# unirestore/UniRestore

Measured on AMD Instinct MI355X. Metric: restored 512x512 images/sec @ 20 denoise steps (whole job), higher is better.
Workload: dtype bf16; 1 GPU; PIR 512x512 batch=8/GPU, 20 DDIM steps, bf16, hipGraph replay (BASELINE.json configs[1]; configs[2] shape for N=8); global_batch=8, per_gpu_batch=8, image=512, denoise_steps=20, parallelism=image-parallel dp1, weights=seeded random init (no checkpoints reachable)

## Files before the change

### unirestore_amd/csrc/tchain.hip

```cpp
#include "common.h"
#include "tchain_asm.inc"

namespace {

constexpr int TC_WB = 40960;
constexpr int TC_AUX = 4096;
constexpr int TC_TILE = TC_WB + TC_AUX;
constexpr int TC_SHARE = TC_TILE / 4;
constexpr int TC_NS = 3;
constexpr int TC_TOK = 128;
constexpr int TC_LDS = TC_NS * TC_TILE;

typedef __attribute__((address_space(3))) void* lptr_t;
typedef __attribute__((ext_vector_type(4))) unsigned u32x4;

#define TC_WAIT(N) asm volatile("s_waitcnt vmcnt(%0) lgkmcnt(0)" ::"n"(N) : "memory")

__device__ __forceinline__ float f4e(const float4& v, int e) { return e == 0 ? v.x : e == 1 ? v.y : e == 2 ? v.z : v.w; }

template <int NF> __device__ __forceinline__ void zero_acc(f32x16 (&acc)[NF]) {
#pragma unroll
  for (int f = 0; f < NF; ++f)
#pragma unroll
    for (int e = 0; e < 16; ++e) acc[f][e] = 0.f;
}

template <bool F16>
struct TChain {
  typedef typename Frag<F16>::type frag_t;
  unsigned lds0;
  u32x4 rs;
  int lane, wid, h, voff;
  int ti, ntiles, islot, cslot;
  int aoff[4];

#define TC_MFMA_BLOCK(ASM, ...)                                                              \
  do {                                                                                       \
    if constexpr (F16) asm volatile(ASM("v_mfma_f32_32x32x16_f16") __VA_ARGS__);              \
    else asm volatile(ASM("v_mfma_f32_32x32x16_bf16") __VA_ARGS__);                           \
  } while (0)

  __device__ __forceinline__ void init(unsigned char* sm, const unsigned char* stream, int nt) {
    lds0 = __builtin_amdgcn_readfirstlane((unsigned)(uintptr_t)(lptr_t)sm);
    lane = threadIdx.x & 63;
    wid = __builtin_amdgcn_readfirstlane(threadIdx.x >> 6);
    h = lane >> 5;
    voff = lane * 16;
    ti = islot = cslot = 0;
    ntiles = nt;
    const unsigned long long a = (unsigned long long)stream;
    rs[0] = __builtin_amdgcn_readfirstlane((unsigned)a);
    rs[1] = __builtin_amdgcn_readfirstlane((unsigned)(a >> 32) & 0xffffu);
    rs[2] = 0x7fffffffu;
    rs[3] = 0x00020000u;
#pragma unroll
    for (int s = 0; s < 4; ++s) aoff[s] = (lane & 31) * 128 + ((((2 * s + h) ^ ((lane >> 1) & 7))) << 4);
    dma_alone();
    dma_alone();
  }
  __device__ __forceinline__ void dma_args(unsigned& so, unsigned& ld) {
    const int t = ti < ntiles ? ti : ntiles - 1;
    so = (unsigned)t * TC_TILE + (unsigned)wid * TC_SHARE;
    ld = lds0 + (unsigned)islot * TC_TILE + (unsigned)wid * TC_SHARE;
    ++ti;
    islot = islot == TC_NS - 1 ? 0 : islot + 1;
  }
  __device__ __forceinline__ void dma_alone() {
    unsigned so, ld;
    dma_args(so, ld);
    asm volatile(TC_ASM_DMA : "+s"(so), "+s"(ld) : "v"(voff), "s"(rs) : "memory", "scc");
  }
  template <int EXTRA = 0>
  __device__ __forceinline__ unsigned acquire() {
    TC_WAIT(11 + EXTRA);
    __builtin_amdgcn_s_barrier();
    const unsigned slot = lds0 + (unsigned)cslot * TC_TILE;
    cslot = cslot == TC_NS - 1 ? 0 : cslot + 1;
    return slot;
  }
  __device__ __forceinline__ void drain() {
    TC_WAIT(0);
    __builtin_amdgcn_s_barrier();
  }

  template <bool Z>
  __device__ __forceinline__ void gemm_tile(f32x16 (&acc)[10], const frag_t& b0, const frag_t& b1, const frag_t& b2, const frag_t& b3, unsigned slot) {
    const unsigned a0 = slot + aoff[0], a1 = slot + aoff[1], a2 = slot + aoff[2], a3 = slot + aoff[3];
    frag_t t0, t1, t2, t3, t4, t5, t6;
    unsigned so, ld;
    dma_args(so, ld);
#define TC_GEMM_OPERANDS                                                                                                        \
    : "+a"(acc[0]), "+a"(acc[1]), "+a"(acc[2]), "+a"(acc[3]), "+a"(acc[4]), "+a"(acc[5]), "+a"(acc[6]), "+a"(acc[7]), "+a"(acc[8]),  \
      "+a"(acc[9]), "=&v"(t0), "=&v"(t1), "=&v"(t2), "=&v"(t3), "=&v"(t4), "=&v"(t5), "=&v"(t6), "+s"(so), "+s"(ld)       \
    : "v"(b0), "v"(b1), "v"(b2), "v"(b3), "v"(a0), "v"(a1), "v"(a2), "v"(a3), "v"(voff), "s"(rs), "s"(wid)                                  \
    : "memory", "scc"
    if constexpr (Z) TC_MFMA_BLOCK(TC_ASM_GEMM_N10_Z, TC_GEMM_OPERANDS);
    else TC_MFMA_BLOCK(TC_ASM_GEMM_N10, TC_GEMM_OPERANDS);
#undef TC_GEMM_OPERANDS
  }
  template <int EXTRA = 0>
  __device__ __forceinline__ unsigned gemm_stage(f32x16 (&acc)[10], const frag_t (&xb)[20]) {
    unsigned slot = acquire<EXTRA>();
    gemm_tile<true>(acc, xb[0], xb[1], xb[2], xb[3], slot);
#pragma unroll
    for (int kt = 1; kt < 5; ++kt) {
      slot = kt == 1 ? acquire<EXTRA>() : acquire();
      gemm_tile<false>(acc, xb[4 * kt], xb[4 * kt + 1], xb[4 * kt + 2], xb[4 * kt + 3], slot);
    }
    return slot;
  }
  __device__ __forceinline__ void ff1_tile(f32x16 (&ag)[2], const frag_t (&xb)[20], unsigned slot) {
    const unsigned a0 = slot + aoff[0], a1 = slot + aoff[1], a2 = slot + aoff[2], a3 = slot + aoff[3];
    frag_t t0, t1, t2, t3, t4, t5, t6;
    unsigned so, ld;
    dma_args(so, ld);
    TC_MFMA_BLOCK(TC_ASM_FF1_A,
                  : "+a"(ag[0]), "+a"(ag[1]), "=&v"(t0), "=&v"(t1), "=&v"(t2), "=&v"(t3), "=&v"(t4), "=&v"(t5), "=&v"(t6),
                    "+s"(so), "+s"(ld)
                  : "v"(xb[0]), "v"(xb[1]), "v"(xb[2]), "v"(xb[3]), "v"(xb[4]), "v"(xb[5]), "v"(xb[6]), "v"(xb[7]), "v"(xb[8]), "v"(xb[9]),
                    "v"(xb[10]), "v"(xb[11]), "v"(a0), "v"(a1), "v"(a2), "v"(a3), "v"(voff), "s"(rs), "s"(wid)
                  : "memory", "scc");
    TC_MFMA_BLOCK(TC_ASM_FF1_B,
                  : "+a"(ag[0]), "+a"(ag[1]), "=&v"(t0), "=&v"(t1), "=&v"(t2), "=&v"(t3), "=&v"(t4), "=&v"(t5), "=&v"(t6)
                  : "v"(xb[12]), "v"(xb[13]), "v"(xb[14]), "v"(xb[15]), "v"(xb[16]), "v"(xb[17]), "v"(xb[18]), "v"(xb[19]),
                    "v"(a0), "v"(a1), "v"(a2), "v"(a3)
                  : "memory");
  }

  __device__ __forceinline__ unsigned aux_base(unsigned slot) const { return slot + TC_WB + 32 * h; }
  template <int U>
  __device__ __forceinline__ void aux_ff1(unsigned slot, float4 (&q)[8]) const {
    asm volatile(TC_ASM_AUX_FF1
                 : "=&v"(q[0]), "=&v"(q[1]), "=&v"(q[2]), "=&v"(q[3]), "=&v"(q[4]), "=&v"(q[5]), "=&v"(q[6]), "=&v"(q[7])
                 : "v"(aux_base(slot)), "i"(64 * U)
                 : "memory");
  }
  template <int VEC, int F0>
  __device__ __forceinline__ void aux_vec4(unsigned slot, float4 (&q)[8]) const {
    asm volatile(TC_ASM_AUX_8
                 : "=&v"(q[0]), "=&v"(q[1]), "=&v"(q[2]), "=&v"(q[3]), "=&v"(q[4]), "=&v"(q[5]), "=&v"(q[6]), "=&v"(q[7])
                 : "v"(aux_base(slot)), "i"((VEC + 32 * F0) * 4)
                 : "memory");
  }

  __device__ __forceinline__ void att_s(f32x16& s0, f32x16& s1, f32x16& s2, const frag_t& q0, const frag_t& q1, const frag_t& q2, const frag_t& q3, unsigned slot) {
    const unsigned a0 = slot + aoff[0], a1 = slot + aoff[1], a2 = slot + aoff[2], a3 = slot + aoff[3];
    frag_t t0, t1, t2, t3, t4, t5, t6;
    unsigned so, ld;
    dma_args(so, ld);
    TC_MFMA_BLOCK(TC_ASM_ATT_S,
                  : "+a"(s0), "+a"(s1), "+a"(s2), "=&v"(t0), "=&v"(t1), "=&v"(t2), "=&v"(t3), "=&v"(t4), "=&v"(t5), "=&v"(t6), "+s"(so), "+s"(ld)
                  : "v"(q0), "v"(q1), "v"(q2), "v"(q3), "v"(a0), "v"(a1), "v"(a2), "v"(a3), "v"(voff), "s"(rs), "s"(wid)
                  : "memory", "scc");
  }
  __device__ __forceinline__ void att_pv(f32x16 (&o)[2], const frag_t (&pf)[5], unsigned slot) {
    const unsigned v0 = slot + 12288, v1 = slot + 20480;
    const unsigned a0 = v0 + aoff[0], a1 = v0 + aoff[1], a2 = v0 + aoff[2], a3 = v0 + aoff[3], a4 = v1 + aoff[0];
    frag_t t0, t1, t2, t3, t4, t5, t6;
    TC_MFMA_BLOCK(TC_ASM_ATT_PV,
                  : "+a"(o[0]), "+a"(o[1]), "=&v"(t0), "=&v"(t1), "=&v"(t2), "=&v"(t3), "=&v"(t4), "=&v"(t5), "=&v"(t6)
                  : "v"(pf[0]), "v"(pf[1]), "v"(pf[2]), "v"(pf[3]), "v"(pf[4]), "v"(a0), "v"(a1), "v"(a2), "v"(a3), "v"(a4)
                  : "memory");
  }
  template <int F>
  __device__ __forceinline__ void aux_bc(unsigned slot, float4 (&q)[8]) const {
    asm volatile(TC_ASM_AUX_BC8
                 : "=&v"(q[0]), "=&v"(q[1]), "=&v"(q[2]), "=&v"(q[3]), "=&v"(q[4]), "=&v"(q[5]), "=&v"(q[6]), "=&v"(q[7])
                 : "v"(aux_base(slot)), "i"(128 * F)
                 : "memory");
  }
  template <int FA>
  __device__ __forceinline__ void ln_pack(const f32x16& acc, unsigned slot, float mean, float rstd, frag_t& o0, frag_t& o1) const {
    float4 q[8];
    aux_bc<FA>(slot, q);
    const float mr = mean * rstd;
#pragma unroll
    for (int u = 0; u < 2; ++u) {
      float v[8];
#pragma unroll
      for (int e = 0; e < 8; ++e) v[e] = fmaf(rstd, acc[8 * u + e], fmaf(-mr, f4e(q[4 + 2 * u + (e >> 2)], e & 3), f4e(q[2 * u + (e >> 2)], e & 3)));
      if (u == 0) o0 = pack(v); else o1 = pack(v);
    }
  }

  static __device__ __forceinline__ void unpack(const frag_t& f, float (&o)[8]) { unpack8t<F16>(__builtin_bit_cast(uint4, f), o); }
  static __device__ __forceinline__ frag_t pack(const float (&v)[8]) { return __builtin_bit_cast(frag_t, pack8t<F16>(v)); }

  template <bool RES, bool GELU = false>
  __device__ __forceinline__ void bias_res_pack(const f32x16 (&acc)[10], unsigned slot, const frag_t (&res)[20], frag_t (&out)[20]) const {
    bias_res_pair<RES, GELU, 0>(acc, slot, res, out);
    bias_res_pair<RES, GELU, 1>(acc, slot, res, out);
    bias_res_pair<RES, GELU, 2>(acc, slot, res, out);
    bias_res_pair<RES, GELU, 3>(acc, slot, res, out);
    bias_res_pair<RES, GELU, 4>(acc, slot, res, out);
  }
  template <bool RES, bool GELU, int FP>
  __device__ __forceinline__ void bias_res_pair(const f32x16 (&acc)[10], unsigned slot, const frag_t (&res)[20], frag_t (&out)[20]) const {
    float4 q[8];
    aux_vec4<0, 2 * FP>(slot, q);
#pragma unroll
    for (int i = 0; i < 4; ++i) {
      const int f = 2 * FP + (i >> 1), u = i & 1;
      float r[8], v[8];
      if constexpr (RES) unpack(res[2 * f + u], r);
#pragma unroll
      for (int e = 0; e < 8; ++e) {
        v[e] = acc[f][8 * u + e] + f4e(q[2 * i + (e >> 2)], e & 3);
        if constexpr (GELU) v[e] = gelu_f(v[e]);
        if constexpr (RES) v[e] += r[e];
      }
      out[2 * f + u] = pack(v);
    }
  }
};

template <bool F16, int KS>
__device__ __forceinline__ void row_stats(const typename Frag<F16>::type (&x)[KS], float eps, float& mean, float& rstd) {
  float s = 0.f;
#pragma unroll
  for (int k = 0; k < KS; ++k) {
    float v[8];
    TChain<F16>::unpack(x[k], v);
    s += ((v[0] + v[1]) + (v[2] + v[3])) + ((v[4] + v[5]) + (v[6] + v[7]));
  }
  s += __shfl_xor(s, 32, 64);
  mean = s * (1.0f / (16 * KS));
  float q = 0.f;
#pragma unroll
  for (int k = 0; k < KS; ++k) {
    float v[8];
    TChain<F16>::unpack(x[k], v);
#pragma unroll
    for (int e = 0; e < 8; ++e) { const float d = v[e] - mean; q = fmaf(d, d, q); }
  }
  q += __shfl_xor(q, 32, 64);
  rstd = rsqrtf(q * (1.0f / (16 * KS)) + eps);
}

template <bool F16, int U>
__device__ __forceinline__ typename Frag<F16>::type ff1_epilogue(const TChain<F16>& tc, const f32x16 (&ag)[2], unsigned slot, float rstd, float mr) {
  float4 q[8];
  tc.template aux_ff1<U>(slot, q);
  float v[8];
#pragma unroll
  for (int e = 0; e < 8; ++e) {
    const float ba = f4e(q[e >> 2], e & 3), bg = f4e(q[2 + (e >> 2)], e & 3);
    const float ca = f4e(q[4 + (e >> 2)], e & 3), cg = f4e(q[6 + (e >> 2)], e & 3);
    const float a = fmaf(rstd, ag[0][8 * U + e], fmaf(-mr, ca, ba));
    const float g = fmaf(rstd, ag[1][8 * U + e], fmaf(-mr, cg, bg));
    v[e] = a * gelu_f(g);
  }
  return TChain<F16>::pack(v);
}

template <bool F16>
__device__ __forceinline__ unsigned ff_stage(TChain<F16>& tc, f32x16 (&acc)[10], f32x16 (&ag)[2], const typename Frag<F16>::type (&xb)[20],
                                             float mean, float rstd, int nchunk) {
  typedef typename Frag<F16>::type frag_t;
  const float mr = mean * rstd;
  unsigned last = 0;
  for (int c = 0; c < nchunk; ++c) {
    frag_t hid[4];
#pragma unroll
    for (int half = 0; half < 2; ++half) {
      const unsigned slot = tc.acquire();
      tc.ff1_tile(ag, xb, slot);
      hid[half * 2] = ff1_epilogue<F16, 0>(tc, ag, slot, rstd, mr);
      __builtin_amdgcn_sched_barrier(0);
      hid[half * 2 + 1] = ff1_epilogue<F16, 1>(tc, ag, slot, rstd, mr);
      __builtin_amdgcn_sched_barrier(0);
    }
    last = tc.acquire();
    tc.template gemm_tile<false>(acc, hid[0], hid[1], hid[2], hid[3], last);
  }
  return last;
}

template <bool F16>
__device__ __forceinline__ void load_frags(const uint16_t* __restrict__ base, long long tok, int ld, int h, typename Frag<F16>::type (&x)[20]) {
  const uint16_t* xp = base + tok * ld + 8 * h;
#pragma unroll
  for (int s = 0; s < 20; ++s) x[s] = *reinterpret_cast<const typename Frag<F16>::type*>(xp + 16 * s);
}
#define TC_STORE16(ptr, val) (*reinterpret_cast<uint4*>(ptr) = __builtin_bit_cast(uint4, val))
template <bool F16>
__device__ __forceinline__ void store_frags(uint16_t* __restrict__ base, long long tok, int ld, int h, const typename Frag<F16>::type (&x)[20]) {
  uint16_t* xp = base + tok * ld + 8 * h;
#pragma unroll
  for (int s = 0; s < 20; ++s) TC_STORE16(xp + 16 * s, x[s]);
}

struct MlpP {
  const unsigned char* stream;
  const uint16_t* x;
  uint16_t* y;
  int T, ldx, ldy, ntiles, hidden;
  float eps;
};

template <bool F16>
__global__ __launch_bounds__(256, 1) void tchain_mlp_kernel(const MlpP p) {
  typedef typename Frag<F16>::type frag_t;
  extern __shared__ __attribute__((aligned(16))) unsigned char smem[];
  TChain<F16> tc;
  tc.init(smem, p.stream, p.ntiles);
  const long long tok = (long long)blockIdx.x * TC_TOK + tc.wid * 32 + (tc.lane & 31);
  frag_t xb[20];
  load_frags<F16>(p.x, tok, p.ldx, tc.h, xb);
  float mean, rstd;
  row_stats<F16, 20>(xb, p.eps, mean, rstd);
  f32x16 acc[10], ag[2];
  zero_acc(acc);
  zero_acc(ag);
  const unsigned last = ff_stage<F16>(tc, acc, ag, xb, mean, rstd, p.hidden / 64);
#pragma unroll
  for (int s = 0; s < 20; ++s) asm volatile("" : "+v"(xb[s]));
  tc.template bias_res_pack<true>(acc, last, xb, xb);
  store_frags<F16>(p.y, tok, p.ldy, tc.h, xb);
  TC_WAIT(0);
}

template <bool F16>
int launch_mlp(const MlpP& p, hipStream_t s) {
  static ur::DeviceOnce attr_once;
  if (auto once_guard = attr_once.first()) {
    hipFuncSetAttribute(reinterpret_cast<const void*>(&tchain_mlp_kernel<F16>), hipFuncAttributeMaxDynamicSharedMemorySize, TC_LDS);
  }
  hipLaunchKernelGGL((tchain_mlp_kernel<F16>), dim3(p.T / TC_TOK), dim3(256), TC_LDS, s, p);
  return ur::check_launch("ur_ff_geglu_fused");
}


__device__ __forceinline__ long long token_again() {
  unsigned t = threadIdx.x;
  asm volatile("" : "+v"(t));
  return (long long)blockIdx.x * TC_TOK + (t >> 6) * 32 + (t & 31);
}

template <bool F16>
__device__ __forceinline__ void launder(typename Frag<F16>::type (&x)[20]) {
#pragma unroll
  for (int s = 0; s < 20; ++s) asm volatile("" : "+v"(x[s]));
}

template <bool F16, int F>
__device__ __forceinline__ void head_out(const TChain<F16>& tc, const f32x16 (&acc)[10], unsigned slot, float mean, float rstd, int part,
                                         uint16_t* op, typename Frag<F16>::type (&xb)[20]) {
  typedef typename Frag<F16>::type frag_t;
  frag_t o0, o1;
  tc.template ln_pack<F>(acc[F], slot, mean, rstd, o0, o1);
  if (part < 2) {
    TC_STORE16(op + 32 * F, o0);
    TC_STORE16(op + 32 * F + 16, o1);
  } else {
    xb[2 * F] = o0;
    xb[2 * F + 1] = o1;
  }
}

struct HeadP {
  const unsigned char* stream;
  const uint16_t* x;
  const float* ab;
  uint16_t* h0;
  uint16_t* q;
  uint16_t* k;
  uint16_t* vt;
  int T, tok_per_img, ntiles;
  float eps;
};

template <bool F16>
__global__ __launch_bounds__(256, 1) void tchain_head_kernel(const HeadP p) {
  typedef typename Frag<F16>::type frag_t;
  constexpr int C = 320;
  extern __shared__ __attribute__((aligned(16))) unsigned char smem[];
  TChain<F16> tc;
  tc.init(smem, p.stream, p.ntiles);
  const long long tok0 = (long long)blockIdx.x * TC_TOK;
  const long long tok = tok0 + tc.wid * 32 + (tc.lane & 31);
  const int img = (int)(tok0 / p.tok_per_img);
  frag_t xb[20];
  load_frags<F16>(p.x, tok, C, tc.h, xb);
  {
    const float* ap = p.ab + (long long)img * 2 * C + 8 * tc.h;
#pragma unroll
    for (int s = 0; s < 20; ++s) {
      const float4 a0 = *reinterpret_cast<const float4*>(ap + 16 * s), a1 = *reinterpret_cast<const float4*>(ap + 16 * s + 4);
      const float4 b0 = *reinterpret_cast<const float4*>(ap + C + 16 * s), b1 = *reinterpret_cast<const float4*>(ap + C + 16 * s + 4);
      float v[8];
      tc.unpack(xb[s], v);
      v[0] = fmaf(v[0], a0.x, b0.x); v[1] = fmaf(v[1], a0.y, b0.y); v[2] = fmaf(v[2], a0.z, b0.z); v[3] = fmaf(v[3], a0.w, b0.w);
      v[4] = fmaf(v[4], a1.x, b1.x); v[5] = fmaf(v[5], a1.y, b1.y); v[6] = fmaf(v[6], a1.z, b1.z); v[7] = fmaf(v[7], a1.w, b1.w);
      xb[s] = tc.pack(v);
      if ((s & 3) == 3) __builtin_amdgcn_sched_barrier(0);
    }
  }
  f32x16 acc[10];
  zero_acc(acc);
  unsigned slot = tc.gemm_stage(acc, xb);
  tc.template bias_res_pack<false>(acc, slot, xb, xb);
  store_frags<F16>(p.h0, token_again(), C, tc.h, xb);
  float mean, rstd;
  row_stats<F16, 20>(xb, p.eps, mean, rstd);
  launder<F16>(xb);
#pragma unroll
  for (int part = 0; part < 3; ++part) {
    slot = tc.template gemm_stage<20>(acc, xb);
    uint16_t* op = (part == 0 ? p.q : p.k) + token_again() * C + 8 * tc.h;
    head_out<F16, 0>(tc, acc, slot, mean, rstd, part, op, xb);
    head_out<F16, 1>(tc, acc, slot, mean, rstd, part, op, xb);
    head_out<F16, 2>(tc, acc, slot, mean, rstd, part, op, xb);
    head_out<F16, 3>(tc, acc, slot, mean, rstd, part, op, xb);
    head_out<F16, 4>(tc, acc, slot, mean, rstd, part, op, xb);
    head_out<F16, 5>(tc, acc, slot, mean, rstd, part, op, xb);
    head_out<F16, 6>(tc, acc, slot, mean, rstd, part, op, xb);
    head_out<F16, 7>(tc, acc, slot, mean, rstd, part, op, xb);
    head_out<F16, 8>(tc, acc, slot, mean, rstd, part, op, xb);
    head_out<F16, 9>(tc, acc, slot, mean, rstd, part, op, xb);
  }
  tc.drain();
  unsigned char* tr = smem + tc.wid * (C * 64);
  const int j = tc.lane & 31;
#pragma unroll
  for (int s = 0; s < 20; ++s) {
    const uint4 w = __builtin_bit_cast(uint4, xb[s]);
    const unsigned wv[4] = {w.x, w.y, w.z, w.w};
#pragma unroll
    for (int e = 0; e < 8; ++e) {
      const int c = 16 * s + 8 * tc.h + e;
      *reinterpret_cast<uint16_t*>(tr + c * 64 + j * 2) = (uint16_t)(wv[e >> 1] >> (16 * (e & 1)));
    }
  }
  __syncthreads();
  {
    const long long tin = tok0 - (long long)img * p.tok_per_img + tc.wid * 32;
    uint16_t* vp = p.vt + (long long)img * C * p.tok_per_img + tin + (tc.lane & 3) * 8;
#pragma unroll
    for (int i = 0; i < 20; ++i) {
      const int r = i * 16 + (tc.lane >> 2);
      *reinterpret_cast<uint4*>(vp + (long long)r * p.tok_per_img) = *reinterpret_cast<const uint4*>(tr + r * 64 + (tc.lane & 3) * 16);
    }
  }
}

template <bool F16>
__device__ __forceinline__ void gn_partials_of_tile(const TChain<F16>& tc, unsigned char* smem, const typename Frag<F16>::type (&y)[20],
                                                    float* gn_part, long long tok0, int tok_per_img) {
  typedef typename Frag<F16>::type frag_t;
  constexpr int C = 320, ROW = 2 * C + 16;
  unsigned char* yt = smem + (tc.wid * 32 + (tc.lane & 31)) * ROW + 16 * tc.h;
#pragma unroll
  for (int s = 0; s < 20; ++s) *reinterpret_cast<frag_t*>(yt + 32 * s) = y[s];
  __syncthreads();
  if (threadIdx.x < C / 2) {
    float s0 = 0.f, s1 = 0.f, q0 = 0.f, q1 = 0.f;
    for (int r = 0; r < TC_TOK; ++r) {
      const uint32_t w = *reinterpret_cast<const uint32_t*>(smem + r * ROW + threadIdx.x * 4);
      const float a = Act<F16>::lo(w), b = Act<F16>::hi(w);
      s0 += a; q0 = fmaf(a, a, q0); s1 += b; q1 = fmaf(b, b, q1);
    }
    const int img = (int)(tok0 / tok_per_img), parts = tok_per_img / TC_TOK;
    const int part = (int)((tok0 - (long long)img * tok_per_img) / TC_TOK);
    float* st = gn_part + (((long long)img * parts + part) * C + 2 * threadIdx.x) * 2;
    *reinterpret_cast<float4*>(st) = make_float4(s0, q0, s1, q1);
  }
}

struct CsceP {
  const unsigned char* stream;
  const uint16_t* x;
  const uint16_t* cond;
  uint16_t* y;
  float* gn_part;
  int T, tok_per_img, ntiles;
};

template <bool F16>
__global__ __launch_bounds__(256, 1) void tchain_csce_kernel(const CsceP p) {
  typedef typename Frag<F16>::type frag_t;
  constexpr int C = 320, CC = 256;
  extern __shared__ __attribute__((aligned(16))) unsigned char smem[];
  TChain<F16> tc;
  tc.init(smem, p.stream, p.ntiles);
  const long long tok0 = (long long)blockIdx.x * TC_TOK;
  const long long tok = tok0 + tc.wid * 32 + (tc.lane & 31);
  frag_t sb[20], hb[20];
  {
    const uint16_t* cp = p.cond + tok * CC + 8 * tc.h;
#pragma unroll
    for (int s = 0; s < 16; ++s) hb[s] = *reinterpret_cast<const frag_t*>(cp + 16 * s);
  }
  f32x16 acc[10];
  zero_acc(acc);
  unsigned slot = tc.acquire();
  tc.template gemm_tile<true>(acc, hb[0], hb[1], hb[2], hb[3], slot);
#pragma unroll
  for (int kt = 1; kt < 4; ++kt) {
    slot = tc.acquire();
    tc.template gemm_tile<false>(acc, hb[4 * kt], hb[4 * kt + 1], hb[4 * kt + 2], hb[4 * kt + 3], slot);
    if (kt == 2) load_frags<F16>(p.x, token_again(), C, tc.h, sb);
  }
  tc.template bias_res_pack<true>(acc, slot, sb, sb);
  slot = tc.gemm_stage(acc, sb);
  tc.template bias_res_pack<false, true>(acc, slot, hb, hb);
  slot = tc.gemm_stage(acc, hb);
  tc.template bias_res_pack<true>(acc, slot, sb, sb);
  store_frags<F16>(p.y, token_again(), C, tc.h, sb);
  tc.drain();
  if (p.gn_part) gn_partials_of_tile<F16>(tc, smem, sb, p.gn_part, tok0, p.tok_per_img);
}

struct TailP {
  const unsigned char* stream;
  const uint16_t* o1;
  const uint16_t* h0;
  const uint16_t* xres;
  uint16_t* y;
  float* gn_part;
  int T, tok_per_img, ntiles, hidden, tk;
  float eps, scale_log2e;
};

template <bool F16>
__global__ __launch_bounds__(256, 1) void tchain_tail_kernel(const TailP p) {
  typedef typename Frag<F16>::type frag_t;
  constexpr int C = 320;
  extern __shared__ __attribute__((aligned(16))) unsigned char smem[];
  TChain<F16> tc;
  tc.init(smem, p.stream, p.ntiles);
  const long long tok0 = (long long)blockIdx.x * TC_TOK;
  const long long tok = tok0 + tc.wid * 32 + (tc.lane & 31);
  frag_t hb[20], xq[20];
  load_frags<F16>(p.o1, tok, C, tc.h, xq);
  f32x16 acc[10], ag[2], sc2[1];
  zero_acc(acc);
  zero_acc(ag);
  zero_acc(sc2);
  unsigned slot = tc.acquire();
  tc.template gemm_tile<true>(acc, xq[0], xq[1], xq[2], xq[3], slot);
#pragma unroll
  for (int kt = 1; kt < 5; ++kt) {
    slot = tc.acquire();
    tc.template gemm_tile<false>(acc, xq[4 * kt], xq[4 * kt + 1], xq[4 * kt + 2], xq[4 * kt + 3], slot);
    if (kt == 3) load_frags<F16>(p.h0, token_again(), C, tc.h, hb);
  }
  tc.template bias_res_pack<true>(acc, slot, hb, hb);
  float mean, rstd;
  row_stats<F16, 20>(hb, p.eps, mean, rstd);
  launder<F16>(hb);
#pragma unroll
  for (int hd = 0; hd < 5; ++hd) {
    slot = tc.acquire();
    tc.ff1_tile(ag, hb, slot);
    frag_t qf[4];
    tc.template ln_pack<0>(ag[0], slot, mean, rstd, qf[0], qf[1]);
    tc.template ln_pack<1>(ag[1], slot, mean, rstd, qf[2], qf[3]);
    slot = tc.acquire();
    tc.att_s(ag[0], ag[1], sc2[0], qf[0], qf[1], qf[2], qf[3], slot);
    int lim = p.tk - 8 * tc.h;
    asm volatile("" : "+v"(lim));
    float mx = -INFINITY;
#pragma unroll
    for (int kf = 0; kf < 3; ++kf)
#pragma unroll
      for (int r = 0; r < 16; ++r) {
        const int key = 32 * kf + 16 * (r >> 3) + (r & 7);
        mx = fmaxf(mx, key < lim ? (kf < 2 ? ag[kf & 1][r] : sc2[0][r]) : -INFINITY);
      }
    mx = fmaxf(mx, __shfl_xor(mx, 32, 64));
    const float mc = mx * p.scale_log2e;
    float l = 0.f;
    frag_t pf[5];
#pragma unroll
    for (int ks = 0; ks < 5; ++ks) {
      float v[8];
#pragma unroll
      for (int e = 0; e < 8; ++e) {
        const int key = 16 * ks + e;
        const float sv = ks < 4 ? ag[(ks >> 1) & 1][8 * (ks & 1) + e] : sc2[0][e];
        v[e] = key < lim ? __builtin_amdgcn_exp2f(fmaf(sv, p.scale_log2e, -mc)) : 0.f;
        l += v[e];
      }
      pf[ks] = tc.pack(v);
    }
    l += __shfl_xor(l, 32, 64);
    tc.att_pv(ag, pf, slot);
    const float inv = __builtin_amdgcn_rcpf(l);
    frag_t of[4];
#pragma unroll
    for (int f = 0; f < 2; ++f)
#pragma unroll
      for (int u = 0; u < 2; ++u) {
        float v[8];
#pragma unroll
        for (int e = 0; e < 8; ++e) v[e] = ag[f][8 * u + e] * inv;
        of[2 * f + u] = tc.pack(v);
      }
    slot = tc.acquire();
    if (hd == 0) tc.template gemm_tile<true>(acc, of[0], of[1], of[2], of[3], slot);
    else tc.template gemm_tile<false>(acc, of[0], of[1], of[2], of[3], slot);
  }
  tc.template bias_res_pack<true>(acc, slot, hb, hb);
  row_stats<F16, 20>(hb, p.eps, mean, rstd);
  launder<F16>(hb);
  zero_acc(acc);
  slot = ff_stage<F16>(tc, acc, ag, hb, mean, rstd, p.hidden / 64);
  tc.template bias_res_pack<true>(acc, slot, hb, hb);
  slot = tc.gemm_stage(acc, hb);
  const long long tok2 = token_again();
  load_frags<F16>(p.xres, tok2, C, tc.h, xq);
  tc.template bias_res_pack<true>(acc, slot, xq, xq);
  store_frags<F16>(p.y, tok2, C, tc.h, xq);
  tc.drain();
  if (p.gn_part) gn_partials_of_tile<F16>(tc, smem, xq, p.gn_part, tok0, p.tok_per_img);
}

template <bool F16>
int launch_head(const HeadP& p, hipStream_t s) {
  static ur::DeviceOnce attr_once;
  if (auto once_guard = attr_once.first()) {
    hipFuncSetAttribute(reinterpret_cast<const void*>(&tchain_head_kernel<F16>), hipFuncAttributeMaxDynamicSharedMemorySize, TC_LDS);
  }
  hipLaunchKernelGGL((tchain_head_kernel<F16>), dim3(p.T / TC_TOK), dim3(256), TC_LDS, s, p);
  return ur::check_launch("ur_transformer_head_fused");
}
template <bool F16>
int launch_csce(const CsceP& p, hipStream_t s) {
  static ur::DeviceOnce attr_once;
  if (auto once_guard = attr_once.first()) {
    hipFuncSetAttribute(reinterpret_cast<const void*>(&tchain_csce_kernel<F16>), hipFuncAttributeMaxDynamicSharedMemorySize, TC_LDS);
  }
  hipLaunchKernelGGL((tchain_csce_kernel<F16>), dim3(p.T / TC_TOK), dim3(256), TC_LDS, s, p);
  return ur::check_launch("ur_csce_fused");
}
template <bool F16>
int launch_tail(const TailP& p, hipStream_t s) {
  static ur::DeviceOnce attr_once;
  if (auto once_guard = attr_once.first()) {
    hipFuncSetAttribute(reinterpret_cast<const void*>(&tchain_tail_kernel<F16>), hipFuncAttributeMaxDynamicSharedMemorySize, TC_LDS);
  }
  hipLaunchKernelGGL((tchain_tail_kernel<F16>), dim3(p.T / TC_TOK), dim3(256), TC_LDS, s, p);
  return ur::check_launch("ur_transformer_tail_fused");
}

}

extern "C" size_t ur_chain_tile_bytes(void) { return TC_TILE; }

extern "C" int ur_ff_geglu_fused(const void* x, const void* stream_w, size_t stream_bytes, void* y, long long T, int C, int hidden,
                                 int ldx, int ldy, float ln_eps, int dtype, ur_stream_t stream) {
  UR_REQUIRE(x && stream_w && y, "null pointer");
  UR_REQUIRE_DT(dtype);
  if (C != 320) return ur::fail(UR_E_UNSUPPORTED, "ur_ff_geglu_fused: C must be 320 (token-stationary chain: C/32 accumulator fragments per wave)");
  UR_REQUIRE(T > 0 && T % TC_TOK == 0 && T < (1ll << 31) / (long long)std::max(ldx, ldy), "T must be a positive multiple of 128");
  UR_REQUIRE(hidden > 0 && hidden % 64 == 0 && ldx % 8 == 0 && ldy % 8 == 0 && ldx >= C && ldy >= C, "hidden % 64, ld % 8");
  MlpP p = {};
  p.stream = (const unsigned char*)stream_w; p.x = (const uint16_t*)x; p.y = (uint16_t*)y;
  p.T = (int)T; p.ldx = ldx; p.ldy = ldy; p.hidden = hidden; p.ntiles = 3 * (hidden / 64); p.eps = ln_eps;
  UR_REQUIRE(stream_bytes >= (size_t)p.ntiles * TC_TILE, "weight stream too short");
  hipStream_t s = (hipStream_t)stream;
  const double flops = 2.0 * (double)T * C * hidden * 3.0;
  const double bytes = 2.0 * (double)T * C * 2 + (double)p.ntiles * TC_TILE;
  ur::ProfScope prof("chain_mlp", flops, bytes, s);
  UR_DT_SWITCH(dtype, return (launch_mlp<F16>(p, s)));
  return UR_OK;
}

extern "C" int ur_transformer_head_fused(const void* x, const float* gn_ab, const void* stream_w, size_t stream_bytes, void* h0, void* q,
                                         void* k, void* vt, long long T, int tokens_per_image, int C, float ln_eps, int dtype,
                                         ur_stream_t stream) {
  UR_REQUIRE(x && gn_ab && stream_w && h0 && q && k && vt, "null pointer");
  UR_REQUIRE_DT(dtype);
  if (C != 320) return ur::fail(UR_E_UNSUPPORTED, "ur_transformer_head_fused: C must be 320");
  UR_REQUIRE(T > 0 && tokens_per_image > 0 && tokens_per_image % TC_TOK == 0 && T % tokens_per_image == 0 && T * (long long)C < (1ll << 31),
             "tokens per image must be a multiple of 128 and divide T");
  HeadP p = {};
  p.stream = (const unsigned char*)stream_w; p.x = (const uint16_t*)x; p.ab = gn_ab; p.h0 = (uint16_t*)h0; p.q = (uint16_t*)q;
  p.k = (uint16_t*)k; p.vt = (uint16_t*)vt; p.T = (int)T; p.tok_per_img = tokens_per_image; p.ntiles = 20; p.eps = ln_eps;
  UR_REQUIRE(stream_bytes >= (size_t)p.ntiles * TC_TILE, "weight stream too short");
  hipStream_t s = (hipStream_t)stream;
  ur::ProfScope prof("chain_head", 2.0 * (double)T * C * C * 4.0, 2.0 * (double)T * C * 5 + (double)p.ntiles * TC_TILE, s);
  UR_DT_SWITCH(dtype, return (launch_head<F16>(p, s)));
  return UR_OK;
}

extern "C" int ur_transformer_tail_fused(const void* o1, const void* h0, const void* xres, const void* stream_w, size_t stream_bytes, void* y,
                                         float* gn_part, long long T, int tokens_per_image, int C, int hidden, int heads, int tk,
                                         float ln_eps, float attn_scale, int dtype, ur_stream_t stream) {
  UR_REQUIRE(o1 && h0 && xres && stream_w && y, "null pointer");
  UR_REQUIRE_DT(dtype);
  if (C != 320 || heads != 5 || tk < 1 || tk > 80)
    return ur::fail(UR_E_UNSUPPORTED, "ur_transformer_tail_fused: C must be 320 with 5 heads of 64 and at most 80 context tokens");
  UR_REQUIRE(T > 0 && tokens_per_image > 0 && tokens_per_image % TC_TOK == 0 && T % tokens_per_image == 0 && T * (long long)C < (1ll << 31),
             "tokens per image must be a multiple of 128 and divide T");
  UR_REQUIRE(hidden > 0 && hidden % 64 == 0, "hidden % 64");
  TailP p = {};
  p.stream = (const unsigned char*)stream_w; p.o1 = (const uint16_t*)o1; p.h0 = (const uint16_t*)h0; p.xres = (const uint16_t*)xres;
  p.y = (uint16_t*)y; p.gn_part = gn_part; p.T = (int)T; p.tok_per_img = tokens_per_image; p.hidden = hidden; p.tk = tk;
  p.ntiles = 25 + 3 * (hidden / 64); p.eps = ln_eps; p.scale_log2e = attn_scale * 1.4426950408889634f;
  UR_REQUIRE(stream_bytes >= (size_t)p.ntiles * TC_TILE, "weight stream too short");
  hipStream_t s = (hipStream_t)stream;
  const double flops = 2.0 * (double)T * C * (4.0 * C + 3.0 * hidden) + 4.0 * (double)T * tk * C;
  ur::ProfScope prof("chain_tail", flops, 2.0 * (double)T * C * 4 + (double)p.ntiles * TC_TILE, s);
  UR_DT_SWITCH(dtype, return (launch_tail<F16>(p, s)));
  return UR_OK;
}

extern "C" int ur_csce_fused(const void* x, const void* cond, const void* stream_w, size_t stream_bytes, void* y, float* gn_part, long long T,
                             int tokens_per_image, int C, int Ccond, int dtype, ur_stream_t stream) {
  UR_REQUIRE(x && cond && stream_w && y, "null pointer");
  UR_REQUIRE_DT(dtype);
  if (C != 320 || Ccond != 256) return ur::fail(UR_E_UNSUPPORTED, "ur_csce_fused: C must be 320 and the condition 256 channels wide");
  UR_REQUIRE(T > 0 && tokens_per_image > 0 && tokens_per_image % TC_TOK == 0 && T % tokens_per_image == 0 && T * (long long)C < (1ll << 31),
             "tokens per image must be a multiple of 128 and divide T");
  CsceP p = {};
  p.stream = (const unsigned char*)stream_w; p.x = (const uint16_t*)x; p.cond = (const uint16_t*)cond; p.y = (uint16_t*)y; p.gn_part = gn_part;
  p.T = (int)T; p.tok_per_img = tokens_per_image; p.ntiles = 14;
  UR_REQUIRE(stream_bytes >= (size_t)p.ntiles * TC_TILE, "weight stream too short");
  hipStream_t s = (hipStream_t)stream;
  ur::ProfScope prof("chain_csce", 2.0 * (double)T * C * (Ccond + 2.0 * C), 2.0 * (double)T * (2.0 * C + Ccond) + (double)p.ntiles * TC_TILE, s);
  UR_DT_SWITCH(dtype, return (launch_csce<F16>(p, s)));
  return UR_OK;
}
```

### unirestore_amd/csrc/tchain_asm.inc

```
#pragma once

#define TC_ASM_DMA \
  "s_mov_b32 m0, %1\n\t" \
  "s_nop 0\n\t" \
  "buffer_load_dwordx4 %2, %3, %0 offen offset:0 lds\n\t" \
  "buffer_load_dwordx4 %2, %3, %0 offen offset:1024 lds\n\t" \
  "buffer_load_dwordx4 %2, %3, %0 offen offset:2048 lds\n\t" \
  "buffer_load_dwordx4 %2, %3, %0 offen offset:3072 lds\n\t" \
  "s_add_u32 %0, %0, 0x1000\n\t" \
  "s_add_u32 %1, %1, 0x1000\n\t" \
  "s_mov_b32 m0, %1\n\t" \
  "s_nop 0\n\t" \
  "buffer_load_dwordx4 %2, %3, %0 offen offset:0 lds\n\t" \
  "buffer_load_dwordx4 %2, %3, %0 offen offset:1024 lds\n\t" \
  "buffer_load_dwordx4 %2, %3, %0 offen offset:2048 lds\n\t" \
  "buffer_load_dwordx4 %2, %3, %0 offen offset:3072 lds\n\t" \
  "s_add_u32 %0, %0, 0x1000\n\t" \
  "s_add_u32 %1, %1, 0x1000\n\t" \
  "s_mov_b32 m0, %1\n\t" \
  "s_nop 0\n\t" \
  "buffer_load_dwordx4 %2, %3, %0 offen offset:0 lds\n\t" \
  "buffer_load_dwordx4 %2, %3, %0 offen offset:1024 lds\n\t" \
  "buffer_load_dwordx4 %2, %3, %0 offen offset:2048 lds\n\t"

#define TC_ASM_GEMM_N10(MN) \
  "s_waitcnt lgkmcnt(0)\n\t" \
  "ds_read_b128 %10, %23 offset:0\n\t" \
  "ds_read_b128 %11, %23 offset:4096\n\t" \
  "ds_read_b128 %12, %23 offset:8192\n\t" \
  "ds_read_b128 %13, %23 offset:12288\n\t" \
  "ds_read_b128 %14, %23 offset:16384\n\t" \
  "ds_read_b128 %15, %23 offset:20480\n\t" \
  "ds_read_b128 %16, %23 offset:24576\n\t" \
  "s_waitcnt lgkmcnt(6)\n\t" \
  MN " %0, %10, %19, %0\n\t" \
  "ds_read_b128 %10, %23 offset:28672\n\t" \
  "s_waitcnt lgkmcnt(6)\n\t" \
  MN " %1, %11, %19, %1\n\t" \
  "ds_read_b128 %11, %23 offset:32768\n\t" \
  "s_waitcnt lgkmcnt(6)\n\t" \
  MN " %2, %12, %19, %2\n\t" \
  "ds_read_b128 %12, %23 offset:36864\n\t" \
  "s_waitcnt lgkmcnt(6)\n\t" \
  MN " %3, %13, %19, %3\n\t" \
  "ds_read_b128 %13, %24 offset:0\n\t" \
  "s_waitcnt lgkmcnt(6)\n\t" \
  MN " %4, %14, %19, %4\n\t" \
  "ds_read_b128 %14, %24 offset:4096\n\t" \
  "s_waitcnt lgkmcnt(6)\n\t" \
  MN " %5, %15, %19, %5\n\t" \
  "ds_read_b128 %15, %24 offset:8192\n\t" \
  "s_waitcnt lgkmcnt(6)\n\t" \
  MN " %6, %16, %19, %6\n\t" \
  "ds_read_b128 %16, %24 offset:12288\n\t" \
  "s_waitcnt lgkmcnt(6)\n\t" \
  MN " %7, %10, %19, %7\n\t" \
  "ds_read_b128 %10, %24 offset:16384\n\t" \
  "s_waitcnt lgkmcnt(6)\n\t" \
  MN " %8, %11, %19, %8\n\t" \
  "ds_read_b128 %11, %24 offset:20480\n\t" \
  "s_waitcnt lgkmcnt(6)\n\t" \
  MN " %9, %12, %19, %9\n\t" \
  "ds_read_b128 %12, %24 offset:24576\n\t" \
  "s_cmp_lg_u32 %29, 0\n\t" \
  "s_cbranch_scc1 .Ltc%=_0\n\t" \
  "s_mov_b32 m0, %18\n\t" \
  "s_nop 0\n\t" \
  "buffer_load_dwordx4 %27, %28, %17 offen offset:0 lds\n\t" \
  "buffer_load_dwordx4 %27, %28, %17 offen offset:1024 lds\n\t" \
  "buffer_load_dwordx4 %27, %28, %17 offen offset:2048 lds\n\t" \
  "buffer_load_dwordx4 %27, %28, %17 offen offset:3072 lds\n\t" \
  "s_add_u32 %17, %17, 0x1000\n\t" \
  "s_add_u32 %18, %18, 0x1000\n\t" \
  "s_mov_b32 m0, %18\n\t" \
  "s_nop 0\n\t" \
  "buffer_load_dwordx4 %27, %28, %17 offen offset:0 lds\n\t" \
  "buffer_load_dwordx4 %27, %28, %17 offen offset:1024 lds\n\t" \
  "buffer_load_dwordx4 %27, %28, %17 offen offset:2048 lds\n\t" \
  "buffer_load_dwordx4 %27, %28, %17 offen offset:3072 lds\n\t" \
  "s_add_u32 %17, %17, 0x1000\n\t" \
  "s_add_u32 %18, %18, 0x1000\n\t" \
  "s_mov_b32 m0, %18\n\t" \
  "s_nop 0\n\t" \
  "buffer_load_dwordx4 %27, %28, %17 offen offset:0 lds\n\t" \
  "buffer_load_dwordx4 %27, %28, %17 offen offset:1024 lds\n\t" \
  "buffer_load_dwordx4 %27, %28, %17 offen offset:2048 lds\n\t" \
  ".Ltc%=_0:\n\t" \
  "s_waitcnt lgkmcnt(6)\n\t" \
  MN " %0, %13, %20, %0\n\t" \
  "ds_read_b128 %13, %24 offset:28672\n\t" \
  "s_waitcnt lgkmcnt(6)\n\t" \
  MN " %1, %14, %20, %1\n\t" \
  "ds_read_b128 %14, %24 offset:32768\n\t" \
  "s_waitcnt lgkmcnt(6)\n\t" \
  MN " %2, %15, %20, %2\n\t" \
  "ds_read_b128 %15, %24 offset:36864\n\t" \
  "s_waitcnt lgkmcnt(6)\n\t" \
  MN " %3, %16, %20, %3\n\t" \
  "ds_read_b128 %16, %25 offset:0\n\t" \
  "s_waitcnt lgkmcnt(6)\n\t" \
  MN " %4, %10, %20, %4\n\t" \
  "ds_read_b128 %10, %25 offset:4096\n\t" \
  "s_waitcnt lgkmcnt(6)\n\t" \
  MN " %5, %11, %20, %5\n\t" \
  "ds_read_b128 %11, %25 offset:8192\n\t" \
  "s_waitcnt lgkmcnt(6)\n\t" \
  MN " %6, %12, %20, %6\n\t" \
  "ds_read_b128 %12, %25 offset:12288\n\t" \
  "s_waitcnt lgkmcnt(6)\n\t" \
  MN " %7, %13, %20, %7\n\t" \
  "ds_read_b128 %13, %25 offset:16384\n\t" \
  "s_waitcnt lgkmcnt(6)\n\t" \
  MN " %8, %14, %20, %8\n\t" \
  "ds_read_b128 %14, %25 offset:20480\n\t" \
  "s_waitcnt lgkmcnt(6)\n\t" \
  MN " %9, %15, %20, %9\n\t" \
  "ds_read_b128 %15, %25 offset:24576\n\t" \
  "s_cmp_lg_u32 %29, 1\n\t" \
  "s_cbranch_scc1 .Ltc%=_1\n\t" \
  "s_mov_b32 m0, %18\n\t" \
  "s_nop 0\n\t" \
  "buffer_load_dwordx4 %27, %28, %17 offen offset:0 lds\n\t" \
  "buffer_load_dwordx4 %27, %28, %17 offen offset:1024 lds\n\t" \
  "buffer_load_dwordx4 %27, %28, %17 offen offset:2048 lds\n\t" \
  "buffer_load_dwordx4 %27, %28, %17 offen offset:3072 lds\n\t" \
  "s_add_u32 %17, %17, 0x1000\n\t" \
  "s_add_u32 %18, %18, 0x1000\n\t" \
  "s_mov_b32 m0, %18\n\t" \
  "s_nop 0\n\t" \
  "buffer_load_dwordx4 %27, %28, %17 offen offset:0 lds\n\t" \
  "buffer_load_dwordx4 %27, %28, %17 offen offset:1024 lds\n\t" \
  "buffer_load_dwordx4 %27, %28, %17 offen offset:2048 lds\n\t" \
  "buffer_load_dwordx4 %27, %28, %17 offen offset:3072 lds\n\t" \
  "s_add_u32 %17, %17, 0x1000\n\t" \
  "s_add_u32 %18, %18, 0x1000\n\t" \
  "s_mov_b32 m0, %18\n\t" \
  "s_nop 0\n\t" \
  "buffer_load_dwordx4 %27, %28, %17 offen offset:0 lds\n\t" \
  "buffer_load_dwordx4 %27, %28, %17 offen offset:1024 lds\n\t" \
  "buffer_load_dwordx4 %27, %28, %17 offen offset:2048 lds\n\t" \
  ".Ltc%=_1:\n\t" \
  "s_waitcnt lgkmcnt(6)\n\t" \
  MN " %0, %16, %21, %0\n\t" \
  "ds_read_b128 %16, %25 offset:28672\n\t" \
  "s_waitcnt lgkmcnt(6)\n\t" \
  MN " %1, %10, %21, %1\n\t" \
  "ds_read_b128 %10, %25 offset:32768\n\t" \
  "s_waitcnt lgkmcnt(6)\n\t" \
  MN " %2, %11, %21, %2\n\t" \
  "ds_read_b128 %11, %25 offset:36864\n\t" \
  "s_waitcnt lgkmcnt(6)\n\t" \
  MN " %3, %12, %21, %3\n\t" \
  "ds_read_b128 %12, %26 offset:0\n\t" \
  "s_waitcnt lgkmcnt(6)\n\t" \
  MN " %4, %13, %21, %4\n\t" \
  "ds_read_b128 %13, %26 offset:4096\n\t" \
  "s_waitcnt lgkmcnt(6)\n\t" \
  MN " %5, %14, %21, %5\n\t" \
  "ds_read_b128 %14, %26 offset:8192\n\t" \
  "s_waitcnt lgkmcnt(6)\n\t" \
  MN " %6, %15, %21, %6\n\t" \
  "ds_read_b128 %15, %26 offset:12288\n\t" \
  "s_waitcnt lgkmcnt(6)\n\t" \
  MN " %7, %16, %21, %7\n\t" \
  "ds_read_b128 %16, %26 offset:16384\n\t" \
  "s_waitcnt lgkmcnt(6)\n\t" \
  MN " %8, %10, %21, %8\n\t" \
  "ds_read_b128 %10, %26 offset:20480\n\t" \
  "s_waitcnt lgkmcnt(6)\n\t" \
  MN " %9, %11, %21, %9\n\t" \
  "ds_read_b128 %11, %26 offset:24576\n\t" \
  "s_cmp_lg_u32 %29, 2\n\t" \
  "s_cbranch_scc1 .Ltc%=_2\n\t" \
  "s_mov_b32 m0, %18\n\t" \
  "s_nop 0\n\t" \
  "buffer_load_dwordx4 %27, %28, %17 offen offset:0 lds\n\t" \
  "buffer_load_dwordx4 %27, %28, %17 offen offset:1024 lds\n\t" \
  "buffer_load_dwordx4 %27, %28, %17 offen offset:2048 lds\n\t" \
  "buffer_load_dwordx4 %27, %28, %17 offen offset:3072 lds\n\t" \
  "s_add_u32 %17, %17, 0x1000\n\t" \
  "s_add_u32 %18, %18, 0x1000\n\t" \
  "s_mov_b32 m0, %18\n\t" \
  "s_nop 0\n\t" \
  "buffer_load_dwordx4 %27, %28, %17 offen offset:0 lds\n\t" \
  "buffer_load_dwordx4 %27, %28, %17 offen offset:1024 lds\n\t" \
  "buffer_load_dwordx4 %27, %28, %17 offen offset:2048 lds\n\t" \
  "buffer_load_dwordx4 %27, %28, %17 offen offset:3072 lds\n\t" \
  "s_add_u32 %17, %17, 0x1000\n\t" \
  "s_add_u32 %18, %18, 0x1000\n\t" \
  "s_mov_b32 m0, %18\n\t" \
  "s_nop 0\n\t" \
  "buffer_load_dwordx4 %27, %28, %17 offen offset:0 lds\n\t" \
  "buffer_load_dwordx4 %27, %28, %17 offen offset:1024 lds\n\t" \
  "buffer_load_dwordx4 %27, %28, %17 offen offset:2048 lds\n\t" \
  ".Ltc%=_2:\n\t" \
  "s_waitcnt lgkmcnt(6)\n\t" \
  MN " %0, %12, %22, %0\n\t" \
  "ds_read_b128 %12, %26 offset:28672\n\t" \
  "s_waitcnt lgkmcnt(6)\n\t" \
  MN " %1, %13, %22, %1\n\t" \
  "ds_read_b128 %13, %26 offset:32768\n\t" \
  "s_waitcnt lgkmcnt(6)\n\t" \
  MN " %2, %14, %22, %2\n\t" \
  "ds_read_b128 %14, %26 offset:36864\n\t" \
  "s_waitcnt lgkmcnt(6)\n\t" \
  MN " %3, %15, %22, %3\n\t" \
  "s_waitcnt lgkmcnt(5)\n\t" \
  MN " %4, %16, %22, %4\n\t" \
  "s_waitcnt lgkmcnt(4)\n\t" \
  MN " %5, %10, %22, %5\n\t" \
  "s_waitcnt lgkmcnt(3)\n\t" \
  MN " %6, %11, %22, %6\n\t" \
  "s_waitcnt lgkmcnt(2)\n\t" \
  MN " %7, %12, %22, %7\n\t" \
  "s_waitcnt lgkmcnt(1)\n\t" \
  MN " %8, %13, %22, %8\n\t" \
  "s_waitcnt lgkmcnt(0)\n\t" \
  MN " %9, %14, %22, %9\n\t" \
  "s_cmp_lg_u32 %29, 3\n\t" \
  "s_cbranch_scc1 .Ltc%=_3\n\t" \
  "s_mov_b32 m0, %18\n\t" \
  "s_nop 0\n\t" \
  "buffer_load_dwordx4 %27, %28, %17 offen offset:0 lds\n\t" \
  "buffer_load_dwordx4 %27, %28, %17 offen offset:1024 lds\n\t" \
  "buffer_load_dwordx4 %27, %28, %17 offen offset:2048 lds\n\t" \
  "buffer_load_dwordx4 %27, %28, %17 offen offset:3072 lds\n\t" \
  "s_add_u32 %17, %17, 0x1000\n\t" \
  "s_add_u32 %18, %18, 0x1000\n\t" \
  "s_mov_b32 m0, %18\n\t" \
  "s_nop 0\n\t" \
  "buffer_load_dwordx4 %27, %28, %17 offen offset:0 lds\n\t" \
  "buffer_load_dwordx4 %27, %28, %17 offen offset:1024 lds\n\t" \
  "buffer_load_dwordx4 %27, %28, %17 offen offset:2048 lds\n\t" \
  "buffer_load_dwordx4 %27, %28, %17 offen offset:3072 lds\n\t" \
  "s_add_u32 %17, %17, 0x1000\n\t" \
  "s_add_u32 %18, %18, 0x1000\n\t" \
  "s_mov_b32 m0, %18\n\t" \
  "s_nop 0\n\t" \
  "buffer_load_dwordx4 %27, %28, %17 offen offset:0 lds\n\t" \
  "buffer_load_dwordx4 %27, %28, %17 offen offset:1024 lds\n\t" \
  "buffer_load_dwordx4 %27, %28, %17 offen offset:2048 lds\n\t" \
  ".Ltc%=_3:\n\t" \
  "s_nop 15\n\t"

#define TC_ASM_GEMM_N10_Z(MN) \
  "s_waitcnt lgkmcnt(0)\n\t" \
  "ds_read_b128 %10, %23 offset:0\n\t" \
  "ds_read_b128 %11, %23 offset:4096\n\t" \
  "ds_read_b128 %12, %23 offset:8192\n\t" \
  "ds_read_b128 %13, %23 offset:12288\n\t" \
  "ds_read_b128 %14, %23 offset:16384\n\t" \
  "ds_read_b128 %15, %23 offset:20480\n\t" \
  "ds_read_b128 %16, %23 offset:24576\n\t" \
  "s_waitcnt lgkmcnt(6)\n\t" \
  MN " %0, %10, %19, 0\n\t" \
  "ds_read_b128 %10, %23 offset:28672\n\t" \
  "s_waitcnt lgkmcnt(6)\n\t" \
  MN " %1, %11, %19, 0\n\t" \
  "ds_read_b128 %11, %23 offset:32768\n\t" \
  "s_waitcnt lgkmcnt(6)\n\t" \
  MN " %2, %12, %19, 0\n\t" \
  "ds_read_b128 %12, %23 offset:36864\n\t" \
  "s_waitcnt lgkmcnt(6)\n\t" \
  MN " %3, %13, %19, 0\n\t" \
  "ds_read_b128 %13, %24 offset:0\n\t" \
  "s_waitcnt lgkmcnt(6)\n\t" \
  MN " %4, %14, %19, 0\n\t" \
  "ds_read_b128 %14, %24 offset:4096\n\t" \
  "s_waitcnt lgkmcnt(6)\n\t" \
  MN " %5, %15, %19, 0\n\t" \
  "ds_read_b128 %15, %24 offset:8192\n\t" \
  "s_waitcnt lgkmcnt(6)\n\t" \
  MN " %6, %16, %19, 0\n\t" \
  "ds_read_b128 %16, %24 offset:12288\n\t" \
  "s_waitcnt lgkmcnt(6)\n\t" \
  MN " %7, %10, %19, 0\n\t" \
  "ds_read_b128 %10, %24 offset:16384\n\t" \
  "s_waitcnt lgkmcnt(6)\n\t" \
  MN " %8, %11, %19, 0\n\t" \
  "ds_read_b128 %11, %24 offset:20480\n\t" \
  "s_waitcnt lgkmcnt(6)\n\t" \
  MN " %9, %12, %19, 0\n\t" \
  "ds_read_b128 %12, %24 offset:24576\n\t" \
  "s_cmp_lg_u32 %29, 0\n\t" \
  "s_cbranch_scc1 .Ltc%=_0\n\t" \
  "s_mov_b32 m0, %18\n\t" \
  "s_nop 0\n\t" \
  "buffer_load_dwordx4 %27, %28, %17 offen offset:0 lds\n\t" \
  "buffer_load_dwordx4 %27, %28, %17 offen offset:1024 lds\n\t" \
  "buffer_load_dwordx4 %27, %28, %17 offen offset:2048 lds\n\t" \
  "buffer_load_dwordx4 %27, %28, %17 offen offset:3072 lds\n\t" \
  "s_add_u32 %17, %17, 0x1000\n\t" \
  "s_add_u32 %18, %18, 0x1000\n\t" \
  "s_mov_b32 m0, %18\n\t" \
  "s_nop 0\n\t" \
  "buffer_load_dwordx4 %27, %28, %17 offen offset:0 lds\n\t" \
  "buffer_load_dwordx4 %27, %28, %17 offen offset:1024 lds\n\t" \
  "buffer_load_dwordx4 %27, %28, %17 offen offset:2048 lds\n\t" \
  "buffer_load_dwordx4 %27, %28, %17 offen offset:3072 lds\n\t" \
  "s_add_u32 %17, %17, 0x1000\n\t" \
  "s_add_u32 %18, %18, 0x1000\n\t" \
  "s_mov_b32 m0, %18\n\t" \
  "s_nop 0\n\t" \
  "buffer_load_dwordx4 %27, %28, %17 offen offset:0 lds\n\t" \
  "buffer_load_dwordx4 %27, %28, %17 offen offset:1024 lds\n\t" \
  "buffer_load_dwordx4 %27, %28, %17 offen offset:2048 lds\n\t" \
  ".Ltc%=_0:\n\t" \
  "s_waitcnt lgkmcnt(6)\n\t" \
  MN " %0, %13, %20, %0\n\t" \
  "ds_read_b128 %13, %24 offset:28672\n\t" \
  "s_waitcnt lgkmcnt(6)\n\t" \
  MN " %1, %14, %20, %1\n\t" \
  "ds_read_b128 %14, %24 offset:32768\n\t" \
  "s_waitcnt lgkmcnt(6)\n\t" \
  MN " %2, %15, %20, %2\n\t" \
  "ds_read_b128 %15, %24 offset:36864\n\t" \
  "s_waitcnt lgkmcnt(6)\n\t" \
  MN " %3, %16, %20, %3\n\t" \
  "ds_read_b128 %16, %25 offset:0\n\t" \
  "s_waitcnt lgkmcnt(6)\n\t" \
  MN " %4, %10, %20, %4\n\t" \
  "ds_read_b128 %10, %25 offset:4096\n\t" \
  "s_waitcnt lgkmcnt(6)\n\t" \
  MN " %5, %11, %20, %5\n\t" \
  "ds_read_b128 %11, %25 offset:8192\n\t" \
  "s_waitcnt lgkmcnt(6)\n\t" \
  MN " %6, %12, %20, %6\n\t" \
  "ds_read_b128 %12, %25 offset:12288\n\t" \
  "s_waitcnt lgkmcnt(6)\n\t" \
  MN " %7, %13, %20, %7\n\t" \
  "ds_read_b128 %13, %25 offset:16384\n\t" \
  "s_waitcnt lgkmcnt(6)\n\t" \
  MN " %8, %14, %20, %8\n\t" \
  "ds_read_b128 %14, %25 offset:20480\n\t" \
  "s_waitcnt lgkmcnt(6)\n\t" \
  MN " %9, %15, %20, %9\n\t" \
  "ds_read_b128 %15, %25 offset:24576\n\t" \
  "s_cmp_lg_u32 %29, 1\n\t" \
  "s_cbranch_scc1 .Ltc%=_1\n\t" \
  "s_mov_b32 m0, %18\n\t" \
  "s_nop 0\n\t" \
  "buffer_load_dwordx4 %27, %28, %17 offen offset:0 lds\n\t" \
  "buffer_load_dwordx4 %27, %28, %17 offen offset:1024 lds\n\t" \
  "buffer_load_dwordx4 %27, %28, %17 offen offset:2048 lds\n\t" \
  "buffer_load_dwordx4 %27, %28, %17 offen offset:3072 lds\n\t" \
  "s_add_u32 %17, %17, 0x1000\n\t" \
  "s_add_u32 %18, %18, 0x1000\n\t" \
  "s_mov_b32 m0, %18\n\t" \
  "s_nop 0\n\t" \
  "buffer_load_dwordx4 %27, %28, %17 offen offset:0 lds\n\t" \
  "buffer_load_dwordx4 %27, %28, %17 offen offset:1024 lds\n\t" \
  "buffer_load_dwordx4 %27, %28, %17 offen offset:2048 lds\n\t" \
  "buffer_load_dwordx4 %27, %28, %17 offen offset:3072 lds\n\t" \
  "s_add_u32 %17, %17, 0x1000\n\t" \
  "s_add_u32 %18, %18, 0x1000\n\t" \
  "s_mov_b32 m0, %18\n\t" \
  "s_nop 0\n\t" \
  "buffer_load_dwordx4 %27, %28, %17 offen offset:0 lds\n\t" \
  "buffer_load_dwordx4 %27, %28, %17 offen offset:1024 lds\n\t" \
  "buffer_load_dwordx4 %27, %28, %17 offen offset:2048 lds\n\t" \
  ".Ltc%=_1:\n\t" \
  "s_waitcnt lgkmcnt(6)\n\t" \
  MN " %0, %16, %21, %0\n\t" \
  "ds_read_b128 %16, %25 offset:28672\n\t" \
  "s_waitcnt lgkmcnt(6)\n\t" \
  MN " %1, %10, %21, %1\n\t" \
  "ds_read_b128 %10, %25 offset:32768\n\t" \
  "s_waitcnt lgkmcnt(6)\n\t" \
  MN " %2, %11, %21, %2\n\t" \
  "ds_read_b128 %11, %25 offset:36864\n\t" \
  "s_waitcnt lgkmcnt(6)\n\t" \
  MN " %3, %12, %21, %3\n\t" \
  "ds_read_b128 %12, %26 offset:0\n\t" \
  "s_waitcnt lgkmcnt(6)\n\t" \
  MN " %4, %13, %21, %4\n\t" \
  "ds_read_b128 %13, %26 offset:4096\n\t" \
  "s_waitcnt lgkmcnt(6)\n\t" \
  MN " %5, %14, %21, %5\n\t" \
  "ds_read_b128 %14, %26 offset:8192\n\t" \
  "s_waitcnt lgkmcnt(6)\n\t" \
  MN " %6, %15, %21, %6\n\t" \
  "ds_read_b128 %15, %26 offset:12288\n\t" \
  "s_waitcnt lgkmcnt(6)\n\t" \
  MN " %7, %16, %21, %7\n\t" \
  "ds_read_b128 %16, %26 offset:16384\n\t" \
  "s_waitcnt lgkmcnt(6)\n\t" \
  MN " %8, %10, %21, %8\n\t" \
  "ds_read_b128 %10, %26 offset:20480\n\t" \
  "s_waitcnt lgkmcnt(6)\n\t" \
  MN " %9, %11, %21, %9\n\t" \
  "ds_read_b128 %11, %26 offset:24576\n\t" \
  "s_cmp_lg_u32 %29, 2\n\t" \
  "s_cbranch_scc1 .Ltc%=_2\n\t" \
  "s_mov_b32 m0, %18\n\t" \
  "s_nop 0\n\t" \
  "buffer_load_dwordx4 %27, %28, %17 offen offset:0 lds\n\t" \
  "buffer_load_dwordx4 %27, %28, %17 offen offset:1024 lds\n\t" \
  "buffer_load_dwordx4 %27, %28, %17 offen offset:2048 lds\n\t" \
  "buffer_load_dwordx4 %27, %28, %17 offen offset:3072 lds\n\t" \
  "s_add_u32 %17, %17, 0x1000\n\t" \
  "s_add_u32 %18, %18, 0x1000\n\t" \
  "s_mov_b32 m0, %18\n\t" \
  "s_nop 0\n\t" \
  "buffer_load_dwordx4 %27, %28, %17 offen offset:0 lds\n\t" \
  "buffer_load_dwordx4 %27, %28, %17 offen offset:1024 lds\n\t" \
  "buffer_load_dwordx4 %27, %28, %17 offen offset:2048 lds\n\t" \
  "buffer_load_dwordx4 %27, %28, %17 offen offset:3072 lds\n\t" \
  "s_add_u32 %17, %17, 0x1000\n\t" \
  "s_add_u32 %18, %18, 0x1000\n\t" \
  "s_mov_b32 m0, %18\n\t" \
  "s_nop 0\n\t" \
  "buffer_load_dwordx4 %27, %28, %17 offen offset:0 lds\n\t" \
  "buffer_load_dwordx4 %27, %28, %17 offen offset:1024 lds\n\t" \
  "buffer_load_dwordx4 %27, %28, %17 offen offset:2048 lds\n\t" \
  ".Ltc%=_2:\n\t" \
  "s_waitcnt lgkmcnt(6)\n\t" \
  MN " %0, %12, %22, %0\n\t" \
  "ds_read_b128 %12, %26 offset:28672\n\t" \
  "s_waitcnt lgkmcnt(6)\n\t" \
  MN " %1, %13, %22, %1\n\t" \
  "ds_read_b128 %13, %26 offset:32768\n\t" \
  "s_waitcnt lgkmcnt(6)\n\t" \
  MN " %2, %14, %22, %2\n\t" \
  "ds_read_b128 %14, %26 offset:36864\n\t" \
  "s_waitcnt lgkmcnt(6)\n\t" \
  MN " %3, %15, %22, %3\n\t" \
  "s_waitcnt lgkmcnt(5)\n\t" \
  MN " %4, %16, %22, %4\n\t" \
  "s_waitcnt lgkmcnt(4)\n\t" \
  MN " %5, %10, %22, %5\n\t" \
  "s_waitcnt lgkmcnt(3)\n\t" \
  MN " %6, %11, %22, %6\n\t" \
  "s_waitcnt lgkmcnt(2)\n\t" \
  MN " %7, %12, %22, %7\n\t" \
  "s_waitcnt lgkmcnt(1)\n\t" \
  MN " %8, %13, %22, %8\n\t" \
  "s_waitcnt lgkmcnt(0)\n\t" \
  MN " %9, %14, %22, %9\n\t" \
  "s_cmp_lg_u32 %29, 3\n\t" \
  "s_cbranch_scc1 .Ltc%=_3\n\t" \
  "s_mov_b32 m0, %18\n\t" \
  "s_nop 0\n\t" \
  "buffer_load_dwordx4 %27, %28, %17 offen offset:0 lds\n\t" \
  "buffer_load_dwordx4 %27, %28, %17 offen offset:1024 lds\n\t" \
  "buffer_load_dwordx4 %27, %28, %17 offen offset:2048 lds\n\t" \
  "buffer_load_dwordx4 %27, %28, %17 offen offset:3072 lds\n\t" \
  "s_add_u32 %17, %17, 0x1000\n\t" \
  "s_add_u32 %18, %18, 0x1000\n\t" \
  "s_mov_b32 m0, %18\n\t" \
  "s_nop 0\n\t" \
  "buffer_load_dwordx4 %27, %28, %17 offen offset:0 lds\n\t" \
  "buffer_load_dwordx4 %27, %28, %17 offen offset:1024 lds\n\t" \
  "buffer_load_dwordx4 %27, %28, %17 offen offset:2048 lds\n\t" \
  "buffer_load_dwordx4 %27, %28, %17 offen offset:3072 lds\n\t" \
  "s_add_u32 %17, %17, 0x1000\n\t" \
  "s_add_u32 %18, %18, 0x1000\n\t" \
  "s_mov_b32 m0, %18\n\t" \
  "s_nop 0\n\t" \
  "buffer_load_dwordx4 %27, %28, %17 offen offset:0 lds\n\t" \
  "buffer_load_dwordx4 %27, %28, %17 offen offset:1024 lds\n\t" \
  "buffer_load_dwordx4 %27, %28, %17 offen offset:2048 lds\n\t" \
  ".Ltc%=_3:\n\t" \
  "s_nop 15\n\t"

#define TC_ASM_FF1_A(MN) \
  "s_waitcnt lgkmcnt(0)\n\t" \
  "ds_read_b128 %2, %23 offset:0\n\t" \
  "ds_read_b128 %3, %23 offset:4096\n\t" \
  "ds_read_b128 %4, %24 offset:0\n\t" \
  "ds_read_b128 %5, %24 offset:4096\n\t" \
  "ds_read_b128 %6, %25 offset:0\n\t" \
  "ds_read_b128 %7, %25 offset:4096\n\t" \
  "ds_read_b128 %8, %26 offset:0\n\t" \
  "s_waitcnt lgkmcnt(6)\n\t" \
  MN " %0, %2, %11, 0\n\t" \
  "ds_read_b128 %2, %26 offset:4096\n\t" \
  "s_waitcnt lgkmcnt(6)\n\t" \
  MN " %1, %3, %11, 0\n\t" \
  "ds_read_b128 %3, %23 offset:8192\n\t" \
  "s_waitcnt lgkmcnt(6)\n\t" \
  MN " %0, %4, %12, %0\n\t" \
  "ds_read_b128 %4, %23 offset:12288\n\t" \
  "s_waitcnt lgkmcnt(6)\n\t" \
  MN " %1, %5, %12, %1\n\t" \
  "ds_read_b128 %5, %24 offset:8192\n\t" \
  "s_waitcnt lgkmcnt(6)\n\t" \
  MN " %0, %6, %13, %0\n\t" \
  "ds_read_b128 %6, %24 offset:12288\n\t" \
  "s_waitcnt lgkmcnt(6)\n\t" \
  MN " %1, %7, %13, %1\n\t" \
  "ds_read_b128 %7, %25 offset:8192\n\t" \
  "s_cmp_lg_u32 %29, 0\n\t" \
  "s_cbranch_scc1 .Ltc%=_0\n\t" \
  "s_mov_b32 m0, %10\n\t" \
  "s_nop 0\n\t" \
  "buffer_load_dwordx4 %27, %28, %9 offen offset:0 lds\n\t" \
  "buffer_load_dwordx4 %27, %28, %9 offen offset:1024 lds\n\t" \
  "buffer_load_dwordx4 %27, %28, %9 offen offset:2048 lds\n\t" \
  "buffer_load_dwordx4 %27, %28, %9 offen offset:3072 lds\n\t" \
  "s_add_u32 %9, %9, 0x1000\n\t" \
  "s_add_u32 %10, %10, 0x1000\n\t" \
  "s_mov_b32 m0, %10\n\t" \
  "s_nop 0\n\t" \
  "buffer_load_dwordx4 %27, %28, %9 offen offset:0 lds\n\t" \
  "buffer_load_dwordx4 %27, %28, %9 offen offset:1024 lds\n\t" \
  "buffer_load_dwordx4 %27, %28, %9 offen offset:2048 lds\n\t" \
  "buffer_load_dwordx4 %27, %28, %9 offen offset:3072 lds\n\t" \
  "s_add_u32 %9, %9, 0x1000\n\t" \
  "s_add_u32 %10, %10, 0x1000\n\t" \
  "s_mov_b32 m0, %10\n\t" \
  "s_nop 0\n\t" \
  "buffer_load_dwordx4 %27, %28, %9 offen offset:0 lds\n\t" \
  "buffer_load_dwordx4 %27, %28, %9 offen offset:1024 lds\n\t" \
  "buffer_load_dwordx4 %27, %28, %9 offen offset:2048 lds\n\t" \
  ".Ltc%=_0:\n\t" \
  "s_waitcnt lgkmcnt(6)\n\t" \
  MN " %0, %8, %14, %0\n\t" \
  "ds_read_b128 %8, %25 offset:12288\n\t" \
  "s_waitcnt lgkmcnt(6)\n\t" \
  MN " %1, %2, %14, %1\n\t" \
  "ds_read_b128 %2, %26 offset:8192\n\t" \
  "s_waitcnt lgkmcnt(6)\n\t" \
  MN " %0, %3, %15, %0\n\t" \
  "ds_read_b128 %3, %26 offset:12288\n\t" \
  "s_waitcnt lgkmcnt(6)\n\t" \
  MN " %1, %4, %15, %1\n\t" \
  "ds_read_b128 %4, %23 offset:16384\n\t" \
  "s_waitcnt lgkmcnt(6)\n\t" \
  MN " %0, %5, %16, %0\n\t" \
  "ds_read_b128 %5, %23 offset:20480\n\t" \
  "s_waitcnt lgkmcnt(6)\n\t" \
  MN " %1, %6, %16, %1\n\t" \
  "ds_read_b128 %6, %24 offset:16384\n\t" \
  "s_cmp_lg_u32 %29, 1\n\t" \
  "s_cbranch_scc1 .Ltc%=_1\n\t" \
  "s_mov_b32 m0, %10\n\t" \
  "s_nop 0\n\t" \
  "buffer_load_dwordx4 %27, %28, %9 offen offset:0 lds\n\t" \
  "buffer_load_dwordx4 %27, %28, %9 offen offset:1024 lds\n\t" \
  "buffer_load_dwordx4 %27, %28, %9 offen offset:2048 lds\n\t" \
  "buffer_load_dwordx4 %27, %28, %9 offen offset:3072 lds\n\t" \
  "s_add_u32 %9, %9, 0x1000\n\t" \
  "s_add_u32 %10, %10, 0x1000\n\t" \
  "s_mov_b32 m0, %10\n\t" \
  "s_nop 0\n\t" \
  "buffer_load_dwordx4 %27, %28, %9 offen offset:0 lds\n\t" \
  "buffer_load_dwordx4 %27, %28, %9 offen offset:1024 lds\n\t" \
  "buffer_load_dwordx4 %27, %28, %9 offen offset:2048 lds\n\t" \
  "buffer_load_dwordx4 %27, %28, %9 offen offset:3072 lds\n\t" \
  "s_add_u32 %9, %9, 0x1000\n\t" \
  "s_add_u32 %10, %10, 0x1000\n\t" \
  "s_mov_b32 m0, %10\n\t" \
  "s_nop 0\n\t" \
  "buffer_load_dwordx4 %27, %28, %9 offen offset:0 lds\n\t" \
  "buffer_load_dwordx4 %27, %28, %9 offen offset:1024 lds\n\t" \
  "buffer_load_dwordx4 %27, %28, %9 offen offset:2048 lds\n\t" \
  ".Ltc%=_1:\n\t" \
  "s_waitcnt lgkmcnt(6)\n\t" \
  MN " %0, %7, %17, %0\n\t" \
  "ds_read_b128 %7, %24 offset:20480\n\t" \
  "s_waitcnt lgkmcnt(6)\n\t" \
  MN " %1, %8, %17, %1\n\t" \
  "ds_read_b128 %8, %25 offset:16384\n\t" \
  "s_waitcnt lgkmcnt(6)\n\t" \
  MN " %0, %2, %18, %0\n\t" \
  "ds_read_b128 %2, %25 offset:20480\n\t" \
  "s_waitcnt lgkmcnt(6)\n\t" \
  MN " %1, %3, %18, %1\n\t" \
  "ds_read_b128 %3, %26 offset:16384\n\t" \
  "s_waitcnt lgkmcnt(6)\n\t" \
  MN " %0, %4, %19, %0\n\t" \
  "ds_read_b128 %4, %26 offset:20480\n\t" \
  "s_waitcnt lgkmcnt(6)\n\t" \
  MN " %1, %5, %19, %1\n\t" \
  "s_cmp_lg_u32 %29, 2\n\t" \
  "s_cbranch_scc1 .Ltc%=_2\n\t" \
  "s_mov_b32 m0, %10\n\t" \
  "s_nop 0\n\t" \
  "buffer_load_dwordx4 %27, %28, %9 offen offset:0 lds\n\t" \
  "buffer_load_dwordx4 %27, %28, %9 offen offset:1024 lds\n\t" \
  "buffer_load_dwordx4 %27, %28, %9 offen offset:2048 lds\n\t" \
  "buffer_load_dwordx4 %27, %28, %9 offen offset:3072 lds\n\t" \
  "s_add_u32 %9, %9, 0x1000\n\t" \
  "s_add_u32 %10, %10, 0x1000\n\t" \
  "s_mov_b32 m0, %10\n\t" \
  "s_nop 0\n\t" \
  "buffer_load_dwordx4 %27, %28, %9 offen offset:0 lds\n\t" \
  "buffer_load_dwordx4 %27, %28, %9 offen offset:1024 lds\n\t" \
  "buffer_load_dwordx4 %27, %28, %9 offen offset:2048 lds\n\t" \
  "buffer_load_dwordx4 %27, %28, %9 offen offset:3072 lds\n\t" \
  "s_add_u32 %9, %9, 0x1000\n\t" \
  "s_add_u32 %10, %10, 0x1000\n\t" \
  "s_mov_b32 m0, %10\n\t" \
  "s_nop 0\n\t" \
  "buffer_load_dwordx4 %27, %28, %9 offen offset:0 lds\n\t" \
  "buffer_load_dwordx4 %27, %28, %9 offen offset:1024 lds\n\t" \
  "buffer_load_dwordx4 %27, %28, %9 offen offset:2048 lds\n\t" \
  ".Ltc%=_2:\n\t" \
  "s_waitcnt lgkmcnt(5)\n\t" \
  MN " %0, %6, %20, %0\n\t" \
  "s_waitcnt lgkmcnt(4)\n\t" \
  MN " %1, %7, %20, %1\n\t" \
  "s_waitcnt lgkmcnt(3)\n\t" \
  MN " %0, %8, %21, %0\n\t" \
  "s_waitcnt lgkmcnt(2)\n\t" \
  MN " %1, %2, %21, %1\n\t" \
  "s_waitcnt lgkmcnt(1)\n\t" \
  MN " %0, %3, %22, %0\n\t" \
  "s_waitcnt lgkmcnt(0)\n\t" \
  MN " %1, %4, %22, %1\n\t" \
  "s_cmp_lg_u32 %29, 3\n\t" \
  "s_cbranch_scc1 .Ltc%=_3\n\t" \
  "s_mov_b32 m0, %10\n\t" \
  "s_nop 0\n\t" \
  "buffer_load_dwordx4 %27, %28, %9 offen offset:0 lds\n\t" \
  "buffer_load_dwordx4 %27, %28, %9 offen offset:1024 lds\n\t" \
  "buffer_load_dwordx4 %27, %28, %9 offen offset:2048 lds\n\t" \
  "buffer_load_dwordx4 %27, %28, %9 offen offset:3072 lds\n\t" \
  "s_add_u32 %9, %9, 0x1000\n\t" \
  "s_add_u32 %10, %10, 0x1000\n\t" \
  "s_mov_b32 m0, %10\n\t" \
  "s_nop 0\n\t" \
  "buffer_load_dwordx4 %27, %28, %9 offen offset:0 lds\n\t" \
  "buffer_load_dwordx4 %27, %28, %9 offen offset:1024 lds\n\t" \
  "buffer_load_dwordx4 %27, %28, %9 offen offset:2048 lds\n\t" \
  "buffer_load_dwordx4 %27, %28, %9 offen offset:3072 lds\n\t" \
  "s_add_u32 %9, %9, 0x1000\n\t" \
  "s_add_u32 %10, %10, 0x1000\n\t" \
  "s_mov_b32 m0, %10\n\t" \
  "s_nop 0\n\t" \
  "buffer_load_dwordx4 %27, %28, %9 offen offset:0 lds\n\t" \
  "buffer_load_dwordx4 %27, %28, %9 offen offset:1024 lds\n\t" \
  "buffer_load_dwordx4 %27, %28, %9 offen offset:2048 lds\n\t" \
  ".Ltc%=_3:\n\t"

#define TC_ASM_FF1_B(MN) \
  "s_waitcnt lgkmcnt(0)\n\t" \
  "ds_read_b128 %2, %17 offset:24576\n\t" \
  "ds_read_b128 %3, %17 offset:28672\n\t" \
  "ds_read_b128 %4, %18 offset:24576\n\t" \
  "ds_read_b128 %5, %18 offset:28672\n\t" \
  "ds_read_b128 %6, %19 offset:24576\n\t" \
  "ds_read_b128 %7, %19 offset:28672\n\t" \
  "ds_read_b128 %8, %20 offset:24576\n\t" \
  "s_waitcnt lgkmcnt(6)\n\t" \
  MN " %0, %2, %9, %0\n\t" \
  "ds_read_b128 %2, %20 offset:28672\n\t" \
  "s_waitcnt lgkmcnt(6)\n\t" \
  MN " %1, %3, %9, %1\n\t" \
  "ds_read_b128 %3, %17 offset:32768\n\t" \
  "s_waitcnt lgkmcnt(6)\n\t" \
  MN " %0, %4, %10, %0\n\t" \
  "ds_read_b128 %4, %17 offset:36864\n\t" \
  "s_waitcnt lgkmcnt(6)\n\t" \
  MN " %1, %5, %10, %1\n\t" \
  "ds_read_b128 %5, %18 offset:32768\n\t" \
  "s_waitcnt lgkmcnt(6)\n\t" \
  MN " %0, %6, %11, %0\n\t" \
  "ds_read_b128 %6, %18 offset:36864\n\t" \
  "s_waitcnt lgkmcnt(6)\n\t" \
  MN " %1, %7, %11, %1\n\t" \
  "ds_read_b128 %7, %19 offset:32768\n\t" \
  "s_waitcnt lgkmcnt(6)\n\t" \
  MN " %0, %8, %12, %0\n\t" \
  "ds_read_b128 %8, %19 offset:36864\n\t" \
  "s_waitcnt lgkmcnt(6)\n\t" \
  MN " %1, %2, %12, %1\n\t" \
  "ds_read_b128 %2, %20 offset:32768\n\t" \
  "s_waitcnt lgkmcnt(6)\n\t" \
  MN " %0, %3, %13, %0\n\t" \
  "ds_read_b128 %3, %20 offset:36864\n\t" \
  "s_waitcnt lgkmcnt(6)\n\t" \
  MN " %1, %4, %13, %1\n\t" \
  "s_waitcnt lgkmcnt(5)\n\t" \
  MN " %0, %5, %14, %0\n\t" \
  "s_waitcnt lgkmcnt(4)\n\t" \
  MN " %1, %6, %14, %1\n\t" \
  "s_waitcnt lgkmcnt(3)\n\t" \
  MN " %0, %7, %15, %0\n\t" \
  "s_waitcnt lgkmcnt(2)\n\t" \
  MN " %1, %8, %15, %1\n\t" \
  "s_waitcnt lgkmcnt(1)\n\t" \
  MN " %0, %2, %16, %0\n\t" \
  "s_waitcnt lgkmcnt(0)\n\t" \
  MN " %1, %3, %16, %1\n\t" \
  "s_nop 15\n\t"

#define TC_ASM_ATT_S(MN) \
  "s_waitcnt lgkmcnt(0)\n\t" \
  "ds_read_b128 %3, %16 offset:0\n\t" \
  "ds_read_b128 %4, %16 offset:4096\n\t" \
  "ds_read_b128 %5, %16 offset:8192\n\t" \
  "ds_read_b128 %6, %17 offset:0\n\t" \
  "ds_read_b128 %7, %17 offset:4096\n\t" \
  "ds_read_b128 %8, %17 offset:8192\n\t" \
  "ds_read_b128 %9, %18 offset:0\n\t" \
  "s_waitcnt lgkmcnt(6)\n\t" \
  MN " %0, %3, %12, 0\n\t" \
  "ds_read_b128 %3, %18 offset:4096\n\t" \
  "s_waitcnt lgkmcnt(6)\n\t" \
  MN " %1, %4, %12, 0\n\t" \
  "ds_read_b128 %4, %18 offset:8192\n\t" \
  "s_waitcnt lgkmcnt(6)\n\t" \
  MN " %2, %5, %12, 0\n\t" \
  "ds_read_b128 %5, %19 offset:0\n\t" \
  "s_cmp_lg_u32 %22, 0\n\t" \
  "s_cbranch_scc1 .Ltc%=_0\n\t" \
  "s_mov_b32 m0, %11\n\t" \
  "s_nop 0\n\t" \
  "buffer_load_dwordx4 %20, %21, %10 offen offset:0 lds\n\t" \
  "buffer_load_dwordx4 %20, %21, %10 offen offset:1024 lds\n\t" \
  "buffer_load_dwordx4 %20, %21, %10 offen offset:2048 lds\n\t" \
  "buffer_load_dwordx4 %20, %21, %10 offen offset:3072 lds\n\t" \
  "s_add_u32 %10, %10, 0x1000\n\t" \
  "s_add_u32 %11, %11, 0x1000\n\t" \
  "s_mov_b32 m0, %11\n\t" \
  "s_nop 0\n\t" \
  "buffer_load_dwordx4 %20, %21, %10 offen offset:0 lds\n\t" \
  "buffer_load_dwordx4 %20, %21, %10 offen offset:1024 lds\n\t" \
  "buffer_load_dwordx4 %20, %21, %10 offen offset:2048 lds\n\t" \
  "buffer_load_dwordx4 %20, %21, %10 offen offset:3072 lds\n\t" \
  "s_add_u32 %10, %10, 0x1000\n\t" \
  "s_add_u32 %11, %11, 0x1000\n\t" \
  "s_mov_b32 m0, %11\n\t" \
  "s_nop 0\n\t" \
  "buffer_load_dwordx4 %20, %21, %10 offen offset:0 lds\n\t" \
  "buffer_load_dwordx4 %20, %21, %10 offen offset:1024 lds\n\t" \
  "buffer_load_dwordx4 %20, %21, %10 offen offset:2048 lds\n\t" \
  ".Ltc%=_0:\n\t" \
  "s_waitcnt lgkmcnt(6)\n\t" \
  MN " %0, %6, %13, %0\n\t" \
  "ds_read_b128 %6, %19 offset:4096\n\t" \
  "s_waitcnt lgkmcnt(6)\n\t" \
  MN " %1, %7, %13, %1\n\t" \
  "ds_read_b128 %7, %19 offset:8192\n\t" \
  "s_waitcnt lgkmcnt(6)\n\t" \
  MN " %2, %8, %13, %2\n\t" \
  "s_cmp_lg_u32 %22, 1\n\t" \
  "s_cbranch_scc1 .Ltc%=_1\n\t" \
  "s_mov_b32 m0, %11\n\t" \
  "s_nop 0\n\t" \
  "buffer_load_dwordx4 %20, %21, %10 offen offset:0 lds\n\t" \
  "buffer_load_dwordx4 %20, %21, %10 offen offset:1024 lds\n\t" \
  "buffer_load_dwordx4 %20, %21, %10 offen offset:2048 lds\n\t" \
  "buffer_load_dwordx4 %20, %21, %10 offen offset:3072 lds\n\t" \
  "s_add_u32 %10, %10, 0x1000\n\t" \
  "s_add_u32 %11, %11, 0x1000\n\t" \
  "s_mov_b32 m0, %11\n\t" \
  "s_nop 0\n\t" \
  "buffer_load_dwordx4 %20, %21, %10 offen offset:0 lds\n\t" \
  "buffer_load_dwordx4 %20, %21, %10 offen offset:1024 lds\n\t" \
  "buffer_load_dwordx4 %20, %21, %10 offen offset:2048 lds\n\t" \
  "buffer_load_dwordx4 %20, %21, %10 offen offset:3072 lds\n\t" \
  "s_add_u32 %10, %10, 0x1000\n\t" \
  "s_add_u32 %11, %11, 0x1000\n\t" \
  "s_mov_b32 m0, %11\n\t" \
  "s_nop 0\n\t" \
  "buffer_load_dwordx4 %20, %21, %10 offen offset:0 lds\n\t" \
  "buffer_load_dwordx4 %20, %21, %10 offen offset:1024 lds\n\t" \
  "buffer_load_dwordx4 %20, %21, %10 offen offset:2048 lds\n\t" \
  ".Ltc%=_1:\n\t" \
  "s_waitcnt lgkmcnt(5)\n\t" \
  MN " %0, %9, %14, %0\n\t" \
  "s_waitcnt lgkmcnt(4)\n\t" \
  MN " %1, %3, %14, %1\n\t" \
  "s_waitcnt lgkmcnt(3)\n\t" \
  MN " %2, %4, %14, %2\n\t" \
  "s_cmp_lg_u32 %22, 2\n\t" \
  "s_cbranch_scc1 .Ltc%=_2\n\t" \
  "s_mov_b32 m0, %11\n\t" \
  "s_nop 0\n\t" \
  "buffer_load_dwordx4 %20, %21, %10 offen offset:0 lds\n\t" \
  "buffer_load_dwordx4 %20, %21, %10 offen offset:1024 lds\n\t" \
  "buffer_load_dwordx4 %20, %21, %10 offen offset:2048 lds\n\t" \
  "buffer_load_dwordx4 %20, %21, %10 offen offset:3072 lds\n\t" \
  "s_add_u32 %10, %10, 0x1000\n\t" \
  "s_add_u32 %11, %11, 0x1000\n\t" \
  "s_mov_b32 m0, %11\n\t" \
  "s_nop 0\n\t" \
  "buffer_load_dwordx4 %20, %21, %10 offen offset:0 lds\n\t" \
  "buffer_load_dwordx4 %20, %21, %10 offen offset:1024 lds\n\t" \
  "buffer_load_dwordx4 %20, %21, %10 offen offset:2048 lds\n\t" \
  "buffer_load_dwordx4 %20, %21, %10 offen offset:3072 lds\n\t" \
  "s_add_u32 %10, %10, 0x1000\n\t" \
  "s_add_u32 %11, %11, 0x1000\n\t" \
  "s_mov_b32 m0, %11\n\t" \
  "s_nop 0\n\t" \
  "buffer_load_dwordx4 %20, %21, %10 offen offset:0 lds\n\t" \
  "buffer_load_dwordx4 %20, %21, %10 offen offset:1024 lds\n\t" \
  "buffer_load_dwordx4 %20, %21, %10 offen offset:2048 lds\n\t" \
  ".Ltc%=_2:\n\t" \
  "s_waitcnt lgkmcnt(2)\n\t" \
  MN " %0, %5, %15, %0\n\t" \
  "s_waitcnt lgkmcnt(1)\n\t" \
  MN " %1, %6, %15, %1\n\t" \
  "s_waitcnt lgkmcnt(0)\n\t" \
  MN " %2, %7, %15, %2\n\t" \
  "s_cmp_lg_u32 %22, 3\n\t" \
  "s_cbranch_scc1 .Ltc%=_3\n\t" \
  "s_mov_b32 m0, %11\n\t" \
  "s_nop 0\n\t" \
  "buffer_load_dwordx4 %20, %21, %10 offen offset:0 lds\n\t" \
  "buffer_load_dwordx4 %20, %21, %10 offen offset:1024 lds\n\t" \
  "buffer_load_dwordx4 %20, %21, %10 offen offset:2048 lds\n\t" \
  "buffer_load_dwordx4 %20, %21, %10 offen offset:3072 lds\n\t" \
  "s_add_u32 %10, %10, 0x1000\n\t" \
  "s_add_u32 %11, %11, 0x1000\n\t" \
  "s_mov_b32 m0, %11\n\t" \
  "s_nop 0\n\t" \
  "buffer_load_dwordx4 %20, %21, %10 offen offset:0 lds\n\t" \
  "buffer_load_dwordx4 %20, %21, %10 offen offset:1024 lds\n\t" \
  "buffer_load_dwordx4 %20, %21, %10 offen offset:2048 lds\n\t" \
  "buffer_load_dwordx4 %20, %21, %10 offen offset:3072 lds\n\t" \
  "s_add_u32 %10, %10, 0x1000\n\t" \
  "s_add_u32 %11, %11, 0x1000\n\t" \
  "s_mov_b32 m0, %11\n\t" \
  "s_nop 0\n\t" \
  "buffer_load_dwordx4 %20, %21, %10 offen offset:0 lds\n\t" \
  "buffer_load_dwordx4 %20, %21, %10 offen offset:1024 lds\n\t" \
  "buffer_load_dwordx4 %20, %21, %10 offen offset:2048 lds\n\t" \
  ".Ltc%=_3:\n\t" \
  "s_nop 15\n\t"

#define TC_ASM_ATT_PV(MN) \
  "s_waitcnt lgkmcnt(0)\n\t" \
  "ds_read_b128 %2, %14 offset:0\n\t" \
  "ds_read_b128 %3, %14 offset:4096\n\t" \
  "ds_read_b128 %4, %15 offset:0\n\t" \
  "ds_read_b128 %5, %15 offset:4096\n\t" \
  "ds_read_b128 %6, %16 offset:0\n\t" \
  "ds_read_b128 %7, %16 offset:4096\n\t" \
  "ds_read_b128 %8, %17 offset:0\n\t" \
  "s_waitcnt lgkmcnt(6)\n\t" \
  MN " %0, %2, %9, 0\n\t" \
  "ds_read_b128 %2, %17 offset:4096\n\t" \
  "s_waitcnt lgkmcnt(6)\n\t" \
  MN " %1, %3, %9, 0\n\t" \
  "ds_read_b128 %3, %18 offset:0\n\t" \
  "s_waitcnt lgkmcnt(6)\n\t" \
  MN " %0, %4, %10, %0\n\t" \
  "ds_read_b128 %4, %18 offset:4096\n\t" \
  "s_waitcnt lgkmcnt(6)\n\t" \
  MN " %1, %5, %10, %1\n\t" \
  "s_waitcnt lgkmcnt(5)\n\t" \
  MN " %0, %6, %11, %0\n\t" \
  "s_waitcnt lgkmcnt(4)\n\t" \
  MN " %1, %7, %11, %1\n\t" \
  "s_waitcnt lgkmcnt(3)\n\t" \
  MN " %0, %8, %12, %0\n\t" \
  "s_waitcnt lgkmcnt(2)\n\t" \
  MN " %1, %2, %12, %1\n\t" \
  "s_waitcnt lgkmcnt(1)\n\t" \
  MN " %0, %3, %13, %0\n\t" \
  "s_waitcnt lgkmcnt(0)\n\t" \
  MN " %1, %4, %13, %1\n\t" \
  "s_nop 15\n\t"

#define TC_ASM_AUX_FF1 \
  "ds_read_b128 %0, %8 offset:%c9+0\n\t" \
  "ds_read_b128 %1, %8 offset:%c9+16\n\t" \
  "ds_read_b128 %2, %8 offset:%c9+128\n\t" \
  "ds_read_b128 %3, %8 offset:%c9+144\n\t" \
  "ds_read_b128 %4, %8 offset:%c9+256\n\t" \
  "ds_read_b128 %5, %8 offset:%c9+272\n\t" \
  "ds_read_b128 %6, %8 offset:%c9+384\n\t" \
  "ds_read_b128 %7, %8 offset:%c9+400\n\t" \
  "s_waitcnt lgkmcnt(0)\n\t"

#define TC_ASM_AUX_8 \
  "ds_read_b128 %0, %8 offset:%c9+0\n\t" \
  "ds_read_b128 %1, %8 offset:%c9+16\n\t" \
  "ds_read_b128 %2, %8 offset:%c9+64\n\t" \
  "ds_read_b128 %3, %8 offset:%c9+80\n\t" \
  "ds_read_b128 %4, %8 offset:%c9+128\n\t" \
  "ds_read_b128 %5, %8 offset:%c9+144\n\t" \
  "ds_read_b128 %6, %8 offset:%c9+192\n\t" \
  "ds_read_b128 %7, %8 offset:%c9+208\n\t" \
  "s_waitcnt lgkmcnt(0)\n\t"

#define TC_ASM_AUX_BC8 \
  "ds_read_b128 %0, %8 offset:%c9+0\n\t" \
  "ds_read_b128 %1, %8 offset:%c9+16\n\t" \
  "ds_read_b128 %2, %8 offset:%c9+64\n\t" \
  "ds_read_b128 %3, %8 offset:%c9+80\n\t" \
  "ds_read_b128 %4, %8 offset:%c9+2048\n\t" \
  "ds_read_b128 %5, %8 offset:%c9+2064\n\t" \
  "ds_read_b128 %6, %8 offset:%c9+2112\n\t" \
  "ds_read_b128 %7, %8 offset:%c9+2128\n\t" \
  "s_waitcnt lgkmcnt(0)\n\t"
```

Baseline: 29.38 images/s.

## Interleave FF1 GELU epilogue into next tile's MFMA stream via hand-scheduled asm

Rewrites the feed-forward stage of the fused transformer chain so that the GELU-gated epilogue of one FF1 tile runs inside the inline-asm MFMA loop of the next FF1 tile and of the FF2 tile. Two FF1 accumulator pairs are now held in fixed AGPR ranges, and the bias/mean fold is precomputed into VGPRs. The goal is to hide the VALU epilogue cost, and the serial gaps between matmul tiles, behind matrix-core work. It also adds optional s_memtime instrumentation behind UR_TCHAIN_DBG. The hard-coded register pinning and the clobber lists raise register pressure and add correctness risk.

```diff
diff --git a/unirestore_amd/csrc/tchain.hip b/unirestore_amd/csrc/tchain.hip
--- a/unirestore_amd/csrc/tchain.hip
+++ b/unirestore_amd/csrc/tchain.hip
@@ -33,6 +33,41 @@
   int lane, wid, h, voff;
   int ti, ntiles, islot, cslot;
   int aoff[4];
+
+  enum { TS_TO_OUT, TS_XATT, TS_ACQ, TS_FF1A, TS_EPIA, TS_FF1B, TS_EPIB, TS_FF2, TS_OUT, TS_GN, TS_N };
+#ifdef UR_TCHAIN_DBG
+  unsigned long long dbg_prev, dbg_t0, dbg_rt0;
+  unsigned dbg_sum[TS_N];
+  __device__ __forceinline__ void dbg_init() {
+    asm volatile("s_memrealtime %0\n\ts_memtime %1\n\ts_waitcnt lgkmcnt(0)" : "=s"(dbg_rt0), "=s"(dbg_t0)::"memory");
+    dbg_prev = dbg_t0;
+#pragma unroll
+    for (int k = 0; k < TS_N; ++k) dbg_sum[k] = 0;
+  }
+  __device__ __forceinline__ void dbg_stamp(int k) {
+    unsigned long long now;
+    __builtin_amdgcn_sched_barrier(0);
+    asm volatile("s_memtime %0\n\ts_waitcnt lgkmcnt(0)" : "=s"(now)::"memory");
+    __builtin_amdgcn_sched_barrier(0);
+    dbg_sum[k] += (unsigned)(now - dbg_prev);
+    dbg_prev = now;
+  }
+  __device__ __forceinline__ void dbg_write(uint16_t* row) {
+    unsigned long long now, rt;
+    asm volatile("s_waitcnt vmcnt(0)\n\ts_memrealtime %0\n\ts_memtime %1\n\ts_waitcnt lgkmcnt(0)" : "=s"(rt), "=s"(now)::"memory");
+    if (lane == 0) {
+      unsigned* o = reinterpret_cast<unsigned*>(row);
+#pragma unroll
+      for (int k = 0; k < TS_N; ++k) o[k] = dbg_sum[k];
+      o[TS_N] = (unsigned)(now - dbg_t0);
+      o[TS_N + 1] = (unsigned)(rt - dbg_rt0);
+    }
+  }
+#define TC_STAMP(K) tc.dbg_stamp(TChain<F16>::K)
+#else
+  __device__ __forceinline__ void dbg_init() {}
+#define TC_STAMP(K) ((void)0)
+#endif
 
 #define TC_MFMA_BLOCK(ASM, ...)                                                              \
   do {                                                                                       \
@@ -57,6 +92,7 @@
     for (int s = 0; s < 4; ++s) aoff[s] = (lane & 31) * 128 + ((((2 * s + h) ^ ((lane >> 1) & 7))) << 4);
     dma_alone();
     dma_alone();
+    dbg_init();
   }
   __device__ __forceinline__ void dma_args(unsigned& so, unsigned& ld) {
     const int t = ti < ntiles ? ti : ntiles - 1;
@@ -127,6 +163,53 @@
                   : "memory");
   }
 
+  typedef float f32x8 __attribute__((ext_vector_type(8)));
+  struct FFRegs {
+    f32x16 g0a, g0g, g1a, g1g;
+    f32x8 ta0, ta1, tg0, tg1;
+    frag_t hid0, hid1, hid2, hid3;
+  };
+#define TC_FF_BLOCK(ASM, ...)                                                                        \
+  do {                                                                                               \
+    if constexpr (F16) asm volatile(ASM("v_mfma_f32_32x32x16_f16", "v_cvt_pk_f16_f32") __VA_ARGS__);  \
+    else asm volatile(ASM("v_mfma_f32_32x32x16_bf16", "v_cvt_pk_bf16_f32") __VA_ARGS__);              \
+  } while (0)
+  __device__ __forceinline__ void ff1_first(FFRegs& r, const frag_t (&xb)[20], unsigned slot) {
+    unsigned so, ld;
+    dma_args(so, ld);
+    TC_FF_BLOCK(TC_ASM_FF1_X,
+                : "=&" TC_FF_AG0A(r.g0a), "=&" TC_FF_AG0G(r.g0g), "+s"(so), "+s"(ld)
+                : "v"(xb[0]), "v"(xb[1]), "v"(xb[2]), "v"(xb[3]), "v"(xb[4]), "v"(xb[5]), "v"(xb[6]), "v"(xb[7]), "v"(xb[8]), "v"(xb[9]),
+                  "v"(xb[10]), "v"(xb[11]), "v"(xb[12]), "v"(xb[13]), "v"(xb[14]), "v"(xb[15]), "v"(xb[16]), "v"(xb[17]), "v"(xb[18]),
+                  "v"(xb[19]), "s"(slot), "v"(aoff[0]), "v"(voff), "s"(rs), "s"(wid)
+                : "memory", "scc", TC_FF_CLOBBERS);
+  }
+  __device__ __forceinline__ void ff1_second(FFRegs& r, const frag_t (&xb)[20], unsigned slot, float rstd) {
+    unsigned so, ld;
+    dma_args(so, ld);
+    TC_FF_BLOCK(TC_ASM_FF1_AE,
+                : "=&" TC_FF_AG1A(r.g1a), "=&" TC_FF_AG1G(r.g1g), "=&" TC_FF_HID0(r.hid0), "+s"(so), "+s"(ld)
+                : "v"(xb[0]), "v"(xb[1]), "v"(xb[2]), "v"(xb[3]), "v"(xb[4]), "v"(xb[5]), "v"(xb[6]), "v"(xb[7]), "v"(xb[8]), "v"(xb[9]),
+                  "v"(xb[10]), "v"(xb[11]), "s"(slot), "v"(aoff[0]), "v"(voff), "s"(rs), "s"(wid), TC_FF_AG0A(r.g0a), TC_FF_AG0G(r.g0g),
+                  TC_FF_TA0(r.ta0), TC_FF_TG0(r.tg0), "v"(rstd)
+                : "memory", "scc", TC_FF_CLOBBERS);
+    TC_FF_BLOCK(TC_ASM_FF1_BE,
+                : "+" TC_FF_AG1A(r.g1a), "+" TC_FF_AG1G(r.g1g), "=&" TC_FF_HID1(r.hid1)
+                : "v"(xb[12]), "v"(xb[13]), "v"(xb[14]), "v"(xb[15]), "v"(xb[16]), "v"(xb[17]), "v"(xb[18]), "v"(xb[19]), "s"(slot),
+                  "v"(aoff[0]), TC_FF_AG0A(r.g0a), TC_FF_AG0G(r.g0g), TC_FF_TA1(r.ta1), TC_FF_TG1(r.tg1), "v"(rstd)
+                : "memory", TC_FF_CLOBBERS);
+  }
+  __device__ __forceinline__ void ff2_tile(f32x16 (&acc)[10], FFRegs& r, unsigned slot, float rstd) {
+    unsigned so, ld;
+    dma_args(so, ld);
+    TC_FF_BLOCK(TC_ASM_FF2_E,
+                : "+a"(acc[0]), "+a"(acc[1]), "+a"(acc[2]), "+a"(acc[3]), "+a"(acc[4]), "+a"(acc[5]), "+a"(acc[6]), "+a"(acc[7]), "+a"(acc[8]),
+                  "+a"(acc[9]), "=&" TC_FF_HID2(r.hid2), "=&" TC_FF_HID3(r.hid3), "+s"(so), "+s"(ld)
+                : TC_FF_HID0(r.hid0), TC_FF_HID1(r.hid1), "s"(slot), "v"(aoff[0]), "v"(voff), "s"(rs), "s"(wid), TC_FF_AG1A(r.g1a),
+                  TC_FF_AG1G(r.g1g), TC_FF_TA0(r.ta0), TC_FF_TA1(r.ta1), TC_FF_TG0(r.tg0), TC_FF_TG1(r.tg1), "v"(rstd)
+                : "memory", "scc", TC_FF_CLOBBERS);
+  }
+
   __device__ __forceinline__ unsigned aux_base(unsigned slot) const { return slot + TC_WB + 32 * h; }
   template <int U>
   __device__ __forceinline__ void aux_ff1(unsigned slot, float4 (&q)[8]) const {
@@ -238,41 +321,43 @@
 }
 
 template <bool F16, int U>
-__device__ __forceinline__ typename Frag<F16>::type ff1_epilogue(const TChain<F16>& tc, const f32x16 (&ag)[2], unsigned slot, float rstd, float mr) {
+__device__ __forceinline__ void ff1_fold(const TChain<F16>& tc, unsigned slot, float mr, typename TChain<F16>::f32x8& ta, typename TChain<F16>::f32x8& tg) {
   float4 q[8];
   tc.template aux_ff1<U>(slot, q);
-  float v[8];
 #pragma unroll
   for (int e = 0; e < 8; ++e) {
-    const float ba = f4e(q[e >> 2], e & 3), bg = f4e(q[2 + (e >> 2)], e & 3);
-    const float ca = f4e(q[4 + (e >> 2)], e & 3), cg = f4e(q[6 + (e >> 2)], e & 3);
-    const float a = fmaf(rstd, ag[0][8 * U + e], fmaf(-mr, ca, ba));
-    const float g = fmaf(rstd, ag[1][8 * U + e], fmaf(-mr, cg, bg));
-    v[e] = a * gelu_f(g);
-  }
-  return TChain<F16>::pack(v);
-}
-
-template <bool F16>
-__device__ __forceinline__ unsigned ff_stage(TChain<F16>& tc, f32x16 (&acc)[10], f32x16 (&ag)[2], const typename Frag<F16>::type (&xb)[20],
+    ta[e] = fmaf(-mr, f4e(q[4 + (e >> 2)], e & 3), f4e(q[e >> 2], e & 3));
+    tg[e] = fmaf(-mr, f4e(q[6 + (e >> 2)], e & 3), f4e(q[2 + (e >> 2)], e & 3));
+  }
+}
+
+template <bool F16>
+__device__ __forceinline__ unsigned ff_stage(TChain<F16>& tc, f32x16 (&acc)[10], const typename Frag<F16>::type (&xb)[20],
                                              float mean, float rstd, int nchunk) {
-  typedef typename Frag<F16>::type frag_t;
   const float mr = mean * rstd;
   unsigned last = 0;
   for (int c = 0; c < nchunk; ++c) {
-    frag_t hid[4];
-#pragma unroll
-    for (int half = 0; half < 2; ++half) {
-      const unsigned slot = tc.acquire();
-      tc.ff1_tile(ag, xb, slot);
-      hid[half * 2] = ff1_epilogue<F16, 0>(tc, ag, slot, rstd, mr);
-      __builtin_amdgcn_sched_barrier(0);
-      hid[half * 2 + 1] = ff1_epilogue<F16, 1>(tc, ag, slot, rstd, mr);
-      __builtin_amdgcn_sched_barrier(0);
-    }
+    typename TChain<F16>::FFRegs r;
+    unsigned slot = tc.acquire();
+    TC_STAMP(TS_ACQ);
+    tc.ff1_first(r, xb, slot);
+    TC_STAMP(TS_FF1A);
+    ff1_fold<F16, 0>(tc, slot, mr, r.ta0, r.tg0);
+    ff1_fold<F16, 1>(tc, slot, mr, r.ta1, r.tg1);
+    TC_STAMP(TS_EPIA);
+    slot = tc.acquire();
+    TC_STAMP(TS_ACQ);
+    tc.ff1_second(r, xb, slot, rstd);
+    TC_STAMP(TS_FF1B);
+    ff1_fold<F16, 0>(tc, slot, mr, r.ta0, r.tg0);
+    ff1_fold<F16, 1>(tc, slot, mr, r.ta1, r.tg1);
+    TC_STAMP(TS_EPIB);
     last = tc.acquire();
-    tc.template gemm_tile<false>(acc, hid[0], hid[1], hid[2], hid[3], last);
-  }
+    TC_STAMP(TS_ACQ);
+    tc.ff2_tile(acc, r, last, rstd);
+    TC_STAMP(TS_FF2);
+  }
+  asm volatile("" : "+s"(tc.cslot));
   return last;
 }
 
@@ -309,10 +394,9 @@
   load_frags<F16>(p.x, tok, p.ldx, tc.h, xb);
   float mean, rstd;
   row_stats<F16, 20>(xb, p.eps, mean, rstd);
-  f32x16 acc[10], ag[2];
+  f32x16 acc[10];
   zero_acc(acc);
-  zero_acc(ag);
-  const unsigned last = ff_stage<F16>(tc, acc, ag, xb, mean, rstd, p.hidden / 64);
+  const unsigned last = ff_stage<F16>(tc, acc, xb, mean, rstd, p.hidden / 64);
 #pragma unroll
   for (int s = 0; s < 20; ++s) asm volatile("" : "+v"(xb[s]));
   tc.template bias_res_pack<true>(acc, last, xb, xb);
@@ -546,6 +630,7 @@
     if (kt == 3) load_frags<F16>(p.h0, token_again(), C, tc.h, hb);
   }
   tc.template bias_res_pack<true>(acc, slot, hb, hb);
+  TC_STAMP(TS_TO_OUT);
   float mean, rstd;
   row_stats<F16, 20>(hb, p.eps, mean, rstd);
   launder<F16>(hb);
@@ -605,15 +690,31 @@
   row_stats<F16, 20>(hb, p.eps, mean, rstd);
   launder<F16>(hb);
   zero_acc(acc);
-  slot = ff_stage<F16>(tc, acc, ag, hb, mean, rstd, p.hidden / 64);
+  TC_STAMP(TS_XATT);
+  slot = ff_stage<F16>(tc, acc, hb, mean, rstd, p.hidden / 64);
+  {
+    int a0 = tc.aoff[0];
+    asm volatile("" : "+v"(a0));
+#pragma unroll
+    for (int s = 1; s < 4; ++s) tc.aoff[s] = a0 ^ (s << 5);
+    unsigned t = threadIdx.x;
+    asm volatile("" : "+v"(t));
+    tc.lane = t & 63;
+    tc.h = tc.lane >> 5;
+  }
   tc.template bias_res_pack<true>(acc, slot, hb, hb);
   slot = tc.gemm_stage(acc, hb);
   const long long tok2 = token_again();
   load_frags<F16>(p.xres, tok2, C, tc.h, xq);
   tc.template bias_res_pack<true>(acc, slot, xq, xq);
   store_frags<F16>(p.y, tok2, C, tc.h, xq);
+  TC_STAMP(TS_OUT);
   tc.drain();
   if (p.gn_part) gn_partials_of_tile<F16>(tc, smem, xq, p.gn_part, tok0, p.tok_per_img);
+#ifdef UR_TCHAIN_DBG
+  TC_STAMP(TS_GN);
+  tc.dbg_write(p.y + (tok0 + tc.wid * 32) * C);
+#endif
 }
 
 template <bool F16>
diff --git a/unirestore_amd/csrc/tchain_asm.inc b/unirestore_amd/csrc/tchain_asm.inc
--- a/unirestore_amd/csrc/tchain_asm.inc
+++ b/unirestore_amd/csrc/tchain_asm.inc
@@ -888,3 +888,1186 @@
   "ds_read_b128 %6, %8 offset:%c9+2112\n\t" \
   "ds_read_b128 %7, %8 offset:%c9+2128\n\t" \
   "s_waitcnt lgkmcnt(0)\n\t"
+
+#define TC_ASM_FF1_X(MN, CVT) \
+  "v_add_u32 v224, %24, %25\n\t" \
+  "v_xor_b32 v225, 0x20, %25\n\t" \
+  "v_add_u32 v225, %24, v225\n\t" \
+  "v_xor_b32 v226, 0x40, %25\n\t" \
+  "v_add_u32 v226, %24, v226\n\t" \
+  "v_xor_b32 v227, 0x60, %25\n\t" \
+  "v_add_u32 v227, %24, v227\n\t" \
+  "s_waitcnt lgkmcnt(0)\n\t" \
+  "ds_read_b128 v[228:231], v224 offset:0\n\t" \
+  "ds_read_b128 v[232:235], v224 offset:4096\n\t" \
+  "ds_read_b128 v[236:239], v225 offset:0\n\t" \
+  "ds_read_b128 v[240:243], v225 offset:4096\n\t" \
+  "ds_read_b128 v[244:247], v226 offset:0\n\t" \
+  "ds_read_b128 v[248:251], v226 offset:4096\n\t" \
+  "ds_read_b128 v[252:255], v227 offset:0\n\t" \
+  "s_waitcnt lgkmcnt(6)\n\t" \
+  MN " %0, v[228:231], %4, 0\n\t" \
+  "ds_read_b128 v[228:231], v227 offset:4096\n\t" \
+  "s_waitcnt lgkmcnt(6)\n\t" \
+  MN " %1, v[232:235], %4, 0\n\t" \
+  "ds_read_b128 v[232:235], v224 offset:8192\n\t" \
+  "s_waitcnt lgkmcnt(6)\n\t" \
+  MN " %0, v[236:239], %5, %0\n\t" \
+  "ds_read_b128 v[236:239], v224 offset:12288\n\t" \
+  "s_waitcnt lgkmcnt(6)\n\t" \
+  MN " %1, v[240:243], %5, %1\n\t" \
+  "ds_read_b128 v[240:243], v225 offset:8192\n\t" \
+  "s_waitcnt lgkmcnt(6)\n\t" \
+  MN " %0, v[244:247], %6, %0\n\t" \
+  "ds_read_b128 v[244:247], v225 offset:12288\n\t" \
+  "s_waitcnt lgkmcnt(6)\n\t" \
+  MN " %1, v[248:251], %6, %1\n\t" \
+  "ds_read_b128 v[248:251], v226 offset:8192\n\t" \
+  "s_waitcnt lgkmcnt(6)\n\t" \
+  MN " %0, v[252:255], %7, %0\n\t" \
+  "ds_read_b128 v[252:255], v226 offset:12288\n\t" \
+  "s_waitcnt lgkmcnt(6)\n\t" \
+  MN " %1, v[228:231], %7, %1\n\t" \
+  "ds_read_b128 v[228:231], v227 offset:8192\n\t" \
+  "s_waitcnt lgkmcnt(6)\n\t" \
+  MN " %0, v[232:235], %8, %0\n\t" \
+  "ds_read_b128 v[232:235], v227 offset:12288\n\t" \
+  "s_waitcnt lgkmcnt(6)\n\t" \
+  MN " %1, v[236:239], %8, %1\n\t" \
+  "ds_read_b128 v[236:239], v224 offset:16384\n\t" \
+  "s_cmp_lg_u32 %28, 0\n\t" \
+  "s_cbranch_scc1 .Ltc%=_0\n\t" \
+  "s_mov_b32 m0, %3\n\t" \
+  "s_nop 0\n\t" \
+  "buffer_load_dwordx4 %26, %27, %2 offen offset:0 lds\n\t" \
+  "buffer_load_dwordx4 %26, %27, %2 offen offset:1024 lds\n\t" \
+  "buffer_load_dwordx4 %26, %27, %2 offen offset:2048 lds\n\t" \
+  "buffer_load_dwordx4 %26, %27, %2 offen offset:3072 lds\n\t" \
+  "s_add_u32 %2, %2, 0x1000\n\t" \
+  "s_add_u32 %3, %3, 0x1000\n\t" \
+  "s_mov_b32 m0, %3\n\t" \
+  "s_nop 0\n\t" \
+  "buffer_load_dwordx4 %26, %27, %2 offen offset:0 lds\n\t" \
+  "buffer_load_dwordx4 %26, %27, %2 offen offset:1024 lds\n\t" \
+  "buffer_load_dwordx4 %26, %27, %2 offen offset:2048 lds\n\t" \
+  "buffer_load_dwordx4 %26, %27, %2 offen offset:3072 lds\n\t" \
+  "s_add_u32 %2, %2, 0x1000\n\t" \
+  "s_add_u32 %3, %3, 0x1000\n\t" \
+  "s_mov_b32 m0, %3\n\t" \
+  "s_nop 0\n\t" \
+  "buffer_load_dwordx4 %26, %27, %2 offen offset:0 lds\n\t" \
+  "buffer_load_dwordx4 %26, %27, %2 offen offset:1024 lds\n\t" \
+  "buffer_load_dwordx4 %26, %27, %2 offen offset:2048 lds\n\t" \
+  ".Ltc%=_0:\n\t" \
+  "s_waitcnt lgkmcnt(6)\n\t" \
+  MN " %0, v[240:243], %9, %0\n\t" \
+  "ds_read_b128 v[240:243], v224 offset:20480\n\t" \
+  "s_waitcnt lgkmcnt(6)\n\t" \
+  MN " %1, v[244:247], %9, %1\n\t" \
+  "ds_read_b128 v[244:247], v225 offset:16384\n\t" \
+  "s_waitcnt lgkmcnt(6)\n\t" \
+  MN " %0, v[248:251], %10, %0\n\t" \
+  "ds_read_b128 v[248:251], v225 offset:20480\n\t" \
+  "s_waitcnt lgkmcnt(6)\n\t" \
+  MN " %1, v[252:255], %10, %1\n\t" \
+  "ds_read_b128 v[252:255], v226 offset:16384\n\t" \
+  "s_waitcnt lgkmcnt(6)\n\t" \
+  MN " %0, v[228:231], %11, %0\n\t" \
+  "ds_read_b128 v[228:231], v226 offset:20480\n\t" \
+  "s_waitcnt lgkmcnt(6)\n\t" \
+  MN " %1, v[232:235], %11, %1\n\t" \
+  "ds_read_b128 v[232:235], v227 offset:16384\n\t" \
+  "s_waitcnt lgkmcnt(6)\n\t" \
+  MN " %0, v[236:239], %12, %0\n\t" \
+  "ds_read_b128 v[236:239], v227 offset:20480\n\t" \
+  "s_waitcnt lgkmcnt(6)\n\t" \
+  MN " %1, v[240:243], %12, %1\n\t" \
+  "ds_read_b128 v[240:243], v224 offset:24576\n\t" \
+  "s_waitcnt lgkmcnt(6)\n\t" \
+  MN " %0, v[244:247], %13, %0\n\t" \
+  "ds_read_b128 v[244:247], v224 offset:28672\n\t" \
+  "s_waitcnt lgkmcnt(6)\n\t" \
+  MN " %1, v[248:251], %13, %1\n\t" \
+  "ds_read_b128 v[248:251], v225 offset:24576\n\t" \
+  "s_cmp_lg_u32 %28, 1\n\t" \
+  "s_cbranch_scc1 .Ltc%=_1\n\t" \
+  "s_mov_b32 m0, %3\n\t" \
+  "s_nop 0\n\t" \
+  "buffer_load_dwordx4 %26, %27, %2 offen offset:0 lds\n\t" \
+  "buffer_load_dwordx4 %26, %27, %2 offen offset:1024 lds\n\t" \
+  "buffer_load_dwordx4 %26, %27, %2 offen offset:2048 lds\n\t" \
+  "buffer_load_dwordx4 %26, %27, %2 offen offset:3072 lds\n\t" \
+  "s_add_u32 %2, %2, 0x1000\n\t" \
+  "s_add_u32 %3, %3, 0x1000\n\t" \
+  "s_mov_b32 m0, %3\n\t" \
+  "s_nop 0\n\t" \
+  "buffer_load_dwordx4 %26, %27, %2 offen offset:0 lds\n\t" \
+  "buffer_load_dwordx4 %26, %27, %2 offen offset:1024 lds\n\t" \
+  "buffer_load_dwordx4 %26, %27, %2 offen offset:2048 lds\n\t" \
+  "buffer_load_dwordx4 %26, %27, %2 offen offset:3072 lds\n\t" \
+  "s_add_u32 %2, %2, 0x1000\n\t" \
+  "s_add_u32 %3, %3, 0x1000\n\t" \
+  "s_mov_b32 m0, %3\n\t" \
+  "s_nop 0\n\t" \
+  "buffer_load_dwordx4 %26, %27, %2 offen offset:0 lds\n\t" \
+  "buffer_load_dwordx4 %26, %27, %2 offen offset:1024 lds\n\t" \
+  "buffer_load_dwordx4 %26, %27, %2 offen offset:2048 lds\n\t" \
+  ".Ltc%=_1:\n\t" \
+  "s_waitcnt lgkmcnt(6)\n\t" \
+  MN " %0, v[252:255], %14, %0\n\t" \
+  "ds_read_b128 v[252:255], v225 offset:28672\n\t" \
+  "s_waitcnt lgkmcnt(6)\n\t" \
+  MN " %1, v[228:231], %14, %1\n\t" \
+  "ds_read_b128 v[228:231], v226 offset:24576\n\t" \
+  "s_waitcnt lgkmcnt(6)\n\t" \
+  MN " %0, v[232:235], %15, %0\n\t" \
+  "ds_read_b128 v[232:235], v226 offset:28672\n\t" \
+  "s_waitcnt lgkmcnt(6)\n\t" \
+  MN " %1, v[236:239], %15, %1\n\t" \
+  "ds_read_b128 v[236:239], v227 offset:24576\n\t" \
+  "s_waitcnt lgkmcnt(6)\n\t" \
+  MN " %0, v[240:243], %16, %0\n\t" \
+  "ds_read_b128 v[240:243], v227 offset:28672\n\t" \
+  "s_waitcnt lgkmcnt(6)\n\t" \
+  MN " %1, v[244:247], %16, %1\n\t" \
+  "ds_read_b128 v[244:247], v224 offset:32768\n\t" \
+  "s_waitcnt lgkmcnt(6)\n\t" \
+  MN " %0, v[248:251], %17, %0\n\t" \
+  "ds_read_b128 v[248:251], v224 offset:36864\n\t" \
+  "s_waitcnt lgkmcnt(6)\n\t" \
+  MN " %1, v[252:255], %17, %1\n\t" \
+  "ds_read_b128 v[252:255], v225 offset:32768\n\t" \
+  "s_waitcnt lgkmcnt(6)\n\t" \
+  MN " %0, v[228:231], %18, %0\n\t" \
+  "ds_read_b128 v[228:231], v225 offset:36864\n\t" \
+  "s_waitcnt lgkmcnt(6)\n\t" \
+  MN " %1, v[232:235], %18, %1\n\t" \
+  "ds_read_b128 v[232:235], v226 offset:32768\n\t" \
+  "s_cmp_lg_u32 %28, 2\n\t" \
+  "s_cbranch_scc1 .Ltc%=_2\n\t" \
+  "s_mov_b32 m0, %3\n\t" \
+  "s_nop 0\n\t" \
+  "buffer_load_dwordx4 %26, %27, %2 offen offset:0 lds\n\t" \
+  "buffer_load_dwordx4 %26, %27, %2 offen offset:1024 lds\n\t" \
+  "buffer_load_dwordx4 %26, %27, %2 offen offset:2048 lds\n\t" \
+  "buffer_load_dwordx4 %26, %27, %2 offen offset:3072 lds\n\t" \
+  "s_add_u32 %2, %2, 0x1000\n\t" \
+  "s_add_u32 %3, %3, 0x1000\n\t" \
+  "s_mov_b32 m0, %3\n\t" \
+  "s_nop 0\n\t" \
+  "buffer_load_dwordx4 %26, %27, %2 offen offset:0 lds\n\t" \
+  "buffer_load_dwordx4 %26, %27, %2 offen offset:1024 lds\n\t" \
+  "buffer_load_dwordx4 %26, %27, %2 offen offset:2048 lds\n\t" \
+  "buffer_load_dwordx4 %26, %27, %2 offen offset:3072 lds\n\t" \
+  "s_add_u32 %2, %2, 0x1000\n\t" \
+  "s_add_u32 %3, %3, 0x1000\n\t" \
+  "s_mov_b32 m0, %3\n\t" \
+  "s_nop 0\n\t" \
+  "buffer_load_dwordx4 %26, %27, %2 offen offset:0 lds\n\t" \
+  "buffer_load_dwordx4 %26, %27, %2 offen offset:1024 lds\n\t" \
+  "buffer_load_dwordx4 %26, %27, %2 offen offset:2048 lds\n\t" \
+  ".Ltc%=_2:\n\t" \
+  "s_waitcnt lgkmcnt(6)\n\t" \
+  MN " %0, v[236:239], %19, %0\n\t" \
+  "ds_read_b128 v[236:239], v226 offset:36864\n\t" \
+  "s_waitcnt lgkmcnt(6)\n\t" \
+  MN " %1, v[240:243], %19, %1\n\t" \
+  "ds_read_b128 v[240:243], v227 offset:32768\n\t" \
+  "s_waitcnt lgkmcnt(6)\n\t" \
+  MN " %0, v[244:247], %20, %0\n\t" \
+  "ds_read_b128 v[244:247], v227 offset:36864\n\t" \
+  "s_waitcnt lgkmcnt(6)\n\t" \
+  MN " %1, v[248:251], %20, %1\n\t" \
+  "s_waitcnt lgkmcnt(5)\n\t" \
+  MN " %0, v[252:255], %21, %0\n\t" \
+  "s_waitcnt lgkmcnt(4)\n\t" \
+  MN " %1, v[228:231], %21, %1\n\t" \
+  "s_waitcnt lgkmcnt(3)\n\t" \
+  MN " %0, v[232:235], %22, %0\n\t" \
+  "s_waitcnt lgkmcnt(2)\n\t" \
+  MN " %1, v[236:239], %22, %1\n\t" \
+  "s_waitcnt lgkmcnt(1)\n\t" \
+  MN " %0, v[240:243], %23, %0\n\t" \
+  "s_waitcnt lgkmcnt(0)\n\t" \
+  MN " %1, v[244:247], %23, %1\n\t" \
+  "s_cmp_lg_u32 %28, 3\n\t" \
+  "s_cbranch_scc1 .Ltc%=_3\n\t" \
+  "s_mov_b32 m0, %3\n\t" \
+  "s_nop 0\n\t" \
+  "buffer_load_dwordx4 %26, %27, %2 offen offset:0 lds\n\t" \
+  "buffer_load_dwordx4 %26, %27, %2 offen offset:1024 lds\n\t" \
+  "buffer_load_dwordx4 %26, %27, %2 offen offset:2048 lds\n\t" \
+  "buffer_load_dwordx4 %26, %27, %2 offen offset:3072 lds\n\t" \
+  "s_add_u32 %2, %2, 0x1000\n\t" \
+  "s_add_u32 %3, %3, 0x1000\n\t" \
+  "s_mov_b32 m0, %3\n\t" \
+  "s_nop 0\n\t" \
+  "buffer_load_dwordx4 %26, %27, %2 offen offset:0 lds\n\t" \
+  "buffer_load_dwordx4 %26, %27, %2 offen offset:1024 lds\n\t" \
+  "buffer_load_dwordx4 %26, %27, %2 offen offset:2048 lds\n\t" \
+  "buffer_load_dwordx4 %26, %27, %2 offen offset:3072 lds\n\t" \
+  "s_add_u32 %2, %2, 0x1000\n\t" \
+  "s_add_u32 %3, %3, 0x1000\n\t" \
+  "s_mov_b32 m0, %3\n\t" \
+  "s_nop 0\n\t" \
+  "buffer_load_dwordx4 %26, %27, %2 offen offset:0 lds\n\t" \
+  "buffer_load_dwordx4 %26, %27, %2 offen offset:1024 lds\n\t" \
+  "buffer_load_dwordx4 %26, %27, %2 offen offset:2048 lds\n\t" \
+  ".Ltc%=_3:\n\t" \
+  "s_nop 15\n\t"
+
+#define TC_ASM_FF1_AE(MN, CVT) \
+  "v_add_u32 v224, %17, %18\n\t" \
+  "v_xor_b32 v225, 0x20, %18\n\t" \
+  "v_add_u32 v225, %17, v225\n\t" \
+  "v_xor_b32 v226, 0x40, %18\n\t" \
+  "v_add_u32 v226, %17, v226\n\t" \
+  "v_xor_b32 v227, 0x60, %18\n\t" \
+  "v_add_u32 v227, %17, v227\n\t" \
+  "v_mov_b32 v220, %26\n\t" \
+  "v_mov_b32 v200, 0x41000000\n\t" \
+  "v_mov_b32 v201, 0xc1000000\n\t" \
+  "v_mov_b32 v202, 0xbddaad3c\n\t" \
+  "s_waitcnt lgkmcnt(0)\n\t" \
+  "ds_read_b128 v[228:231], v224 offset:0\n\t" \
+  "ds_read_b128 v[232:235], v224 offset:4096\n\t" \
+  "ds_read_b128 v[236:239], v225 offset:0\n\t" \
+  "ds_read_b128 v[240:243], v225 offset:4096\n\t" \
+  "ds_read_b128 v[244:247], v226 offset:0\n\t" \
+  "ds_read_b128 v[248:251], v226 offset:4096\n\t" \
+  "ds_read_b128 v[252:255], v227 offset:0\n\t" \
+  "s_waitcnt lgkmcnt(6)\n\t" \
+  MN " %0, v[228:231], %5, 0\n\t" \
+  "ds_read_b128 v[228:231], v227 offset:4096\n\t" \
+  "v_accvgpr_read_b32 v204, a208\n\t" \
+  "v_accvgpr_read_b32 v205, a209\n\t" \
+  "v_accvgpr_read_b32 v212, a210\n\t" \
+  "v_accvgpr_read_b32 v213, a211\n\t" \
+  "v_fma_f32 v204, v220, v204, v184\n\t" \
+  "v_fma_f32 v205, v220, v205, v185\n\t" \
+  "s_waitcnt lgkmcnt(6)\n\t" \
+  MN " %1, v[232:235], %5, 0\n\t" \
+  "ds_read_b128 v[232:235], v224 offset:8192\n\t" \
+  "v_fma_f32 v212, v220, v212, v186\n\t" \
+  "v_fma_f32 v213, v220, v213, v187\n\t" \
+  "v_med3_f32 v208, v204, v201, v200\n\t" \
+  "v_med3_f32 v209, v205, v201, v200\n\t" \
+  "v_med3_f32 v216, v212, v201, v200\n\t" \
+  "s_waitcnt lgkmcnt(6)\n\t" \
+  MN " %0, v[236:239], %6, %0\n\t" \
+  "ds_read_b128 v[236:239], v224 offset:12288\n\t" \
+  "v_med3_f32 v217, v213, v201, v200\n\t" \
+  "v_mul_f32 v210, v208, v208\n\t" \
+  "v_mul_f32 v211, v209, v209\n\t" \
+  "v_mul_f32 v218, v216, v216\n\t" \
+  "v_mul_f32 v219, v217, v217\n\t" \
+  "s_waitcnt lgkmcnt(6)\n\t" \
+  MN " %1, v[240:243], %6, %1\n\t" \
+  "ds_read_b128 v[240:243], v225 offset:8192\n\t" \
+  "v_fmamk_f32 v206, v210, 0x3a84f106, v202\n\t" \
+  "v_fmamk_f32 v207, v211, 0x3a84f106, v202\n\t" \
+  "v_fmamk_f32 v214, v218, 0x3a84f106, v202\n\t" \
+  "v_fmamk_f32 v215, v219, 0x3a84f106, v202\n\t" \
+  "v_fmaak_f32 v210, v206, v210, 0xc0134593\n\t" \
+  "s_waitcnt lgkmcnt(6)\n\t" \
+  MN " %0, v[244:247], %7, %0\n\t" \
+  "ds_read_b128 v[244:247], v225 offset:12288\n\t" \
+  "v_fmaak_f32 v211, v207, v211, 0xc0134593\n\t" \
+  "v_fmaak_f32 v218, v214, v218, 0xc0134593\n\t" \
+  "v_fmaak_f32 v219, v215, v219, 0xc0134593\n\t" \
+  "v_mul_f32 v208, v208, v210\n\t" \
+  "v_mul_f32 v209, v209, v211\n\t" \
+  "s_waitcnt lgkmcnt(6)\n\t" \
+  MN " %1, v[248:251], %7, %1\n\t" \
+  "ds_read_b128 v[248:251], v226 offset:8192\n\t" \
+  "s_cmp_lg_u32 %21, 0\n\t" \
+  "s_cbranch_scc1 .Ltc%=_0\n\t" \
+  "s_mov_b32 m0, %4\n\t" \
+  "s_nop 0\n\t" \
+  "buffer_load_dwordx4 %19, %20, %3 offen offset:0 lds\n\t" \
+  "buffer_load_dwordx4 %19, %20, %3 offen offset:1024 lds\n\t" \
+  "buffer_load_dwordx4 %19, %20, %3 offen offset:2048 lds\n\t" \
+  "buffer_load_dwordx4 %19, %20, %3 offen offset:3072 lds\n\t" \
+  "s_add_u32 %3, %3, 0x1000\n\t" \
+  "s_add_u32 %4, %4, 0x1000\n\t" \
+  "s_mov_b32 m0, %4\n\t" \
+  "s_nop 0\n\t" \
+  "buffer_load_dwordx4 %19, %20, %3 offen offset:0 lds\n\t" \
+  "buffer_load_dwordx4 %19, %20, %3 offen offset:1024 lds\n\t" \
+  "buffer_load_dwordx4 %19, %20, %3 offen offset:2048 lds\n\t" \
+  "buffer_load_dwordx4 %19, %20, %3 offen offset:3072 lds\n\t" \
+  "s_add_u32 %3, %3, 0x1000\n\t" \
+  "s_add_u32 %4, %4, 0x1000\n\t" \
+  "s_mov_b32 m0, %4\n\t" \
+  "s_nop 0\n\t" \
+  "buffer_load_dwordx4 %19, %20, %3 offen offset:0 lds\n\t" \
+  "buffer_load_dwordx4 %19, %20, %3 offen offset:1024 lds\n\t" \
+  "buffer_load_dwordx4 %19, %20, %3 offen offset:2048 lds\n\t" \
+  ".Ltc%=_0:\n\t" \
+  "v_mul_f32 v216, v216, v218\n\t" \
+  "v_mul_f32 v217, v217, v219\n\t" \
+  "v_exp_f32 v208, v208\n\t" \
+  "v_exp_f32 v209, v209\n\t" \
+  "v_exp_f32 v216, v216\n\t" \
+  "s_waitcnt lgkmcnt(6)\n\t" \
+  MN " %0, v[252:255], %8, %0\n\t" \
+  "ds_read_b128 v[252:255], v226 offset:12288\n\t" \
+  "v_exp_f32 v217, v217\n\t" \
+  "v_add_f32 v208, 1.0, v208\n\t" \
+  "v_add_f32 v209, 1.0, v209\n\t" \
+  "v_add_f32 v216, 1.0, v216\n\t" \
+  "v_add_f32 v217, 1.0, v217\n\t" \
+  "s_waitcnt lgkmcnt(6)\n\t" \
+  MN " %1, v[228:231], %8, %1\n\t" \
+  "ds_read_b128 v[228:231], v227 offset:8192\n\t" \
+  "v_rcp_f32 v208, v208\n\t" \
+  "v_rcp_f32 v209, v209\n\t" \
+  "v_rcp_f32 v216, v216\n\t" \
+  "v_rcp_f32 v217, v217\n\t" \
+  "v_accvgpr_read_b32 v206, a192\n\t" \
+  "s_waitcnt lgkmcnt(6)\n\t" \
+  MN " %0, v[232:235], %9, %0\n\t" \
+  "ds_read_b128 v[232:235], v227 offset:12288\n\t" \
+  "v_accvgpr_read_b32 v207, a193\n\t" \
+  "v_accvgpr_read_b32 v214, a194\n\t" \
+  "v_accvgpr_read_b32 v215, a195\n\t" \
+  "v_fma_f32 v206, v220, v206, v168\n\t" \
+  "v_fma_f32 v207, v220, v207, v169\n\t" \
+  "s_waitcnt lgkmcnt(6)\n\t" \
+  MN " %1, v[236:239], %9, %1\n\t" \
+  "ds_read_b128 v[236:239], v224 offset:16384\n\t" \
+  "v_fma_f32 v214, v220, v214, v170\n\t" \
+  "v_fma_f32 v215, v220, v215, v171\n\t" \
+  "v_mul_f32 v204, v204, v208\n\t" \
+  "v_mul_f32 v205, v205, v209\n\t" \
+  "v_mul_f32 v212, v212, v216\n\t" \
+  "s_waitcnt lgkmcnt(6)\n\t" \
+  MN " %0, v[240:243], %10, %0\n\t" \
+  "ds_read_b128 v[240:243], v224 offset:20480\n\t" \
+  "v_mul_f32 v213, v213, v217\n\t" \
+  "v_mul_f32 v206, v206, v204\n\t" \
+  "v_mul_f32 v207, v207, v205\n\t" \
+  "v_mul_f32 v214, v214, v212\n\t" \
+  "v_mul_f32 v215, v215, v213\n\t" \
+  "s_waitcnt lgkmcnt(6)\n\t" \
+  MN " %1, v[244:247], %10, %1\n\t" \
+  "ds_read_b128 v[244:247], v225 offset:16384\n\t" \
+  "s_cmp_lg_u32 %21, 1\n\t" \
+  "s_cbranch_scc1 .Ltc%=_1\n\t" \
+  "s_mov_b32 m0, %4\n\t" \
+  "s_nop 0\n\t" \
+  "buffer_load_dwordx4 %19, %20, %3 offen offset:0 lds\n\t" \
+  "buffer_load_dwordx4 %19, %20, %3 offen offset:1024 lds\n\t" \
+  "buffer_load_dwordx4 %19, %20, %3 offen offset:2048 lds\n\t" \
+  "buffer_load_dwordx4 %19, %20, %3 offen offset:3072 lds\n\t" \
+  "s_add_u32 %3, %3, 0x1000\n\t" \
+  "s_add_u32 %4, %4, 0x1000\n\t" \
+  "s_mov_b32 m0, %4\n\t" \
+  "s_nop 0\n\t" \
+  "buffer_load_dwordx4 %19, %20, %3 offen offset:0 lds\n\t" \
+  "buffer_load_dwordx4 %19, %20, %3 offen offset:1024 lds\n\t" \
+  "buffer_load_dwordx4 %19, %20, %3 offen offset:2048 lds\n\t" \
+  "buffer_load_dwordx4 %19, %20, %3 offen offset:3072 lds\n\t" \
+  "s_add_u32 %3, %3, 0x1000\n\t" \
+  "s_add_u32 %4, %4, 0x1000\n\t" \
+  "s_mov_b32 m0, %4\n\t" \
+  "s_nop 0\n\t" \
+  "buffer_load_dwordx4 %19, %20, %3 offen offset:0 lds\n\t" \
+  "buffer_load_dwordx4 %19, %20, %3 offen offset:1024 lds\n\t" \
+  "buffer_load_dwordx4 %19, %20, %3 offen offset:2048 lds\n\t" \
+  ".Ltc%=_1:\n\t" \
+  CVT " v152, v206, v207\n\t" \
+  CVT " v153, v214, v215\n\t" \
+  "v_accvgpr_read_b32 v204, a212\n\t" \
+  "v_accvgpr_read_b32 v205, a213\n\t" \
+  "v_accvgpr_read_b32 v212, a214\n\t" \
+  "s_waitcnt lgkmcnt(6)\n\t" \
+  MN " %0, v[248:251], %11, %0\n\t" \
+  "ds_read_b128 v[248:251], v225 offset:20480\n\t" \
+  "v_accvgpr_read_b32 v213, a215\n\t" \
+  "v_fma_f32 v204, v220, v204, v188\n\t" \
+  "v_fma_f32 v205, v220, v205, v189\n\t" \
+  "v_fma_f32 v212, v220, v212, v190\n\t" \
+  "v_fma_f32 v213, v220, v213, v191\n\t" \
+  "s_waitcnt lgkmcnt(6)\n\t" \
+  MN " %1, v[252:255], %11, %1\n\t" \
+  "ds_read_b128 v[252:255], v226 offset:16384\n\t" \
+  "v_med3_f32 v208, v204, v201, v200\n\t" \
+  "v_med3_f32 v209, v205, v201, v200\n\t" \
+  "v_med3_f32 v216, v212, v201, v200\n\t" \
+  "v_med3_f32 v217, v213, v201, v200\n\t" \
+  "v_mul_f32 v210, v208, v208\n\t" \
+  "s_waitcnt lgkmcnt(6)\n\t" \
+  MN " %0, v[228:231], %12, %0\n\t" \
+  "ds_read_b128 v[228:231], v226 offset:20480\n\t" \
+  "v_mul_f32 v211, v209, v209\n\t" \
+  "v_mul_f32 v218, v216, v216\n\t" \
+  "v_mul_f32 v219, v217, v217\n\t" \
+  "v_fmamk_f32 v206, v210, 0x3a84f106, v202\n\t" \
+  "v_fmamk_f32 v207, v211, 0x3a84f106, v202\n\t" \
+  "s_waitcnt lgkmcnt(6)\n\t" \
+  MN " %1, v[232:235], %12, %1\n\t" \
+  "ds_read_b128 v[232:235], v227 offset:16384\n\t" \
+  "v_fmamk_f32 v214, v218, 0x3a84f106, v202\n\t" \
+  "v_fmamk_f32 v215, v219, 0x3a84f106, v202\n\t" \
+  "v_fmaak_f32 v210, v206, v210, 0xc0134593\n\t" \
+  "v_fmaak_f32 v211, v207, v211, 0xc0134593\n\t" \
+  "v_fmaak_f32 v218, v214, v218, 0xc0134593\n\t" \
+  "s_waitcnt lgkmcnt(6)\n\t" \
+  MN " %0, v[236:239], %13, %0\n\t" \
+  "ds_read_b128 v[236:239], v227 offset:20480\n\t" \
+  "v_fmaak_f32 v219, v215, v219, 0xc0134593\n\t" \
+  "v_mul_f32 v208, v208, v210\n\t" \
+  "v_mul_f32 v209, v209, v211\n\t" \
+  "v_mul_f32 v216, v216, v218\n\t" \
+  "v_mul_f32 v217, v217, v219\n\t" \
+  "s_waitcnt lgkmcnt(6)\n\t" \
+  MN " %1, v[240:243], %13, %1\n\t" \
+  "s_cmp_lg_u32 %21, 2\n\t" \
+  "s_cbranch_scc1 .Ltc%=_2\n\t" \
+  "s_mov_b32 m0, %4\n\t" \
+  "s_nop 0\n\t" \
+  "buffer_load_dwordx4 %19, %20, %3 offen offset:0 lds\n\t" \
+  "buffer_load_dwordx4 %19, %20, %3 offen offset:1024 lds\n\t" \
+  "buffer_load_dwordx4 %19, %20, %3 offen offset:2048 lds\n\t" \
+  "buffer_load_dwordx4 %19, %20, %3 offen offset:3072 lds\n\t" \
+  "s_add_u32 %3, %3, 0x1000\n\t" \
+  "s_add_u32 %4, %4, 0x1000\n\t" \
+  "s_mov_b32 m0, %4\n\t" \
+  "s_nop 0\n\t" \
+  "buffer_load_dwordx4 %19, %20, %3 offen offset:0 lds\n\t" \
+  "buffer_load_dwordx4 %19, %20, %3 offen offset:1024 lds\n\t" \
+  "buffer_load_dwordx4 %19, %20, %3 offen offset:2048 lds\n\t" \
+  "buffer_load_dwordx4 %19, %20, %3 offen offset:3072 lds\n\t" \
+  "s_add_u32 %3, %3, 0x1000\n\t" \
+  "s_add_u32 %4, %4, 0x1000\n\t" \
+  "s_mov_b32 m0, %4\n\t" \
+  "s_nop 0\n\t" \
+  "buffer_load_dwordx4 %19, %20, %3 offen offset:0 lds\n\t" \
+  "buffer_load_dwordx4 %19, %20, %3 offen offset:1024 lds\n\t" \
+  "buffer_load_dwordx4 %19, %20, %3 offen offset:2048 lds\n\t" \
+  ".Ltc%=_2:\n\t" \
+  "v_exp_f32 v208, v208\n\t" \
+  "v_exp_f32 v209, v209\n\t" \
+  "v_exp_f32 v216, v216\n\t" \
+  "v_exp_f32 v217, v217\n\t" \
+  "v_add_f32 v208, 1.0, v208\n\t" \
+  "s_waitcnt lgkmcnt(5)\n\t" \
+  MN " %0, v[244:247], %14, %0\n\t" \
+  "v_add_f32 v209, 1.0, v209\n\t" \
+  "v_add_f32 v216, 1.0, v216\n\t" \
+  "v_add_f32 v217, 1.0, v217\n\t" \
+  "v_rcp_f32 v208, v208\n\t" \
+  "v_rcp_f32 v209, v209\n\t" \
+  "s_waitcnt lgkmcnt(4)\n\t" \
+  MN " %1, v[248:251], %14, %1\n\t" \
+  "v_rcp_f32 v216, v216\n\t" \
+  "v_rcp_f32 v217, v217\n\t" \
+  "v_accvgpr_read_b32 v206, a196\n\t" \
+  "v_accvgpr_read_b32 v207, a197\n\t" \
+  "v_accvgpr_read_b32 v214, a198\n\t" \
+  "s_waitcnt lgkmcnt(3)\n\t" \
+  MN " %0, v[252:255], %15, %0\n\t" \
+  "v_accvgpr_read_b32 v215, a199\n\t" \
+  "v_fma_f32 v206, v220, v206, v172\n\t" \
+  "v_fma_f32 v207, v220, v207, v173\n\t" \
+  "v_fma_f32 v214, v220, v214, v174\n\t" \
+  "v_fma_f32 v215, v220, v215, v175\n\t" \
+  "s_waitcnt lgkmcnt(2)\n\t" \
+  MN " %1, v[228:231], %15, %1\n\t" \
+  "v_mul_f32 v204, v204, v208\n\t" \
+  "v_mul_f32 v205, v205, v209\n\t" \
+  "v_mul_f32 v212, v212, v216\n\t" \
+  "v_mul_f32 v213, v213, v217\n\t" \
+  "v_mul_f32 v206, v206, v204\n\t" \
+  "s_waitcnt lgkmcnt(1)\n\t" \
+  MN " %0, v[232:235], %16, %0\n\t" \
+  "v_mul_f32 v207, v207, v205\n\t" \
+  "v_mul_f32 v214, v214, v212\n\t" \
+  "v_mul_f32 v215, v215, v213\n\t" \
+  CVT " v154, v206, v207\n\t" \
+  CVT " v155, v214, v215\n\t" \
+  "s_waitcnt lgkmcnt(0)\n\t" \
+  MN " %1, v[236:239], %16, %1\n\t" \
+  "s_cmp_lg_u32 %21, 3\n\t" \
+  "s_cbranch_scc1 .Ltc%=_3\n\t" \
+  "s_mov_b32 m0, %4\n\t" \
+  "s_nop 0\n\t" \
+  "buffer_load_dwordx4 %19, %20, %3 offen offset:0 lds\n\t" \
+  "buffer_load_dwordx4 %19, %20, %3 offen offset:1024 lds\n\t" \
+  "buffer_load_dwordx4 %19, %20, %3 offen offset:2048 lds\n\t" \
+  "buffer_load_dwordx4 %19, %20, %3 offen offset:3072 lds\n\t" \
+  "s_add_u32 %3, %3, 0x1000\n\t" \
+  "s_add_u32 %4, %4, 0x1000\n\t" \
+  "s_mov_b32 m0, %4\n\t" \
+  "s_nop 0\n\t" \
+  "buffer_load_dwordx4 %19, %20, %3 offen offset:0 lds\n\t" \
+  "buffer_load_dwordx4 %19, %20, %3 offen offset:1024 lds\n\t" \
+  "buffer_load_dwordx4 %19, %20, %3 offen offset:2048 lds\n\t" \
+  "buffer_load_dwordx4 %19, %20, %3 offen offset:3072 lds\n\t" \
+  "s_add_u32 %3, %3, 0x1000\n\t" \
+  "s_add_u32 %4, %4, 0x1000\n\t" \
+  "s_mov_b32 m0, %4\n\t" \
+  "s_nop 0\n\t" \
+  "buffer_load_dwordx4 %19, %20, %3 offen offset:0 lds\n\t" \
+  "buffer_load_dwordx4 %19, %20, %3 offen offset:1024 lds\n\t" \
+  "buffer_load_dwordx4 %19, %20, %3 offen offset:2048 lds\n\t" \
+  ".Ltc%=_3:\n\t"
+
+#define TC_ASM_FF1_BE(MN, CVT) \
+  "v_add_u32 v224, %11, %12\n\t" \
+  "v_xor_b32 v225, 0x20, %12\n\t" \
+  "v_add_u32 v225, %11, v225\n\t" \
+  "v_xor_b32 v226, 0x40, %12\n\t" \
+  "v_add_u32 v226, %11, v226\n\t" \
+  "v_xor_b32 v227, 0x60, %12\n\t" \
+  "v_add_u32 v227, %11, v227\n\t" \
+  "v_mov_b32 v220, %17\n\t" \
+  "v_mov_b32 v200, 0x41000000\n\t" \
+  "v_mov_b32 v201, 0xc1000000\n\t" \
+  "v_mov_b32 v202, 0xbddaad3c\n\t" \
+  "s_waitcnt lgkmcnt(0)\n\t" \
+  "ds_read_b128 v[228:231], v224 offset:24576\n\t" \
+  "ds_read_b128 v[232:235], v224 offset:28672\n\t" \
+  "ds_read_b128 v[236:239], v225 offset:24576\n\t" \
+  "ds_read_b128 v[240:243], v225 offset:28672\n\t" \
+  "ds_read_b128 v[244:247], v226 offset:24576\n\t" \
+  "ds_read_b128 v[248:251], v226 offset:28672\n\t" \
+  "ds_read_b128 v[252:255], v227 offset:24576\n\t" \
+  "s_waitcnt lgkmcnt(6)\n\t" \
+  MN " %0, v[228:231], %3, %0\n\t" \
+  "ds_read_b128 v[228:231], v227 offset:28672\n\t" \
+  "v_accvgpr_read_b32 v204, a216\n\t" \
+  "v_accvgpr_read_b32 v205, a217\n\t" \
+  "v_accvgpr_read_b32 v212, a218\n\t" \
+  "v_accvgpr_read_b32 v213, a219\n\t" \
+  "v_fma_f32 v204, v220, v204, v192\n\t" \
+  "v_fma_f32 v205, v220, v205, v193\n\t" \
+  "v_fma_f32 v212, v220, v212, v194\n\t" \
+  "v_fma_f32 v213, v220, v213, v195\n\t" \
+  "s_waitcnt lgkmcnt(6)\n\t" \
+  MN " %1, v[232:235], %3, %1\n\t" \
+  "ds_read_b128 v[232:235], v224 offset:32768\n\t" \
+  "v_med3_f32 v208, v204, v201, v200\n\t" \
+  "v_med3_f32 v209, v205, v201, v200\n\t" \
+  "v_med3_f32 v216, v212, v201, v200\n\t" \
+  "v_med3_f32 v217, v213, v201, v200\n\t" \
+  "v_mul_f32 v210, v208, v208\n\t" \
+  "v_mul_f32 v211, v209, v209\n\t" \
+  "v_mul_f32 v218, v216, v216\n\t" \
+  "v_mul_f32 v219, v217, v217\n\t" \
+  "s_waitcnt lgkmcnt(6)\n\t" \
+  MN " %0, v[236:239], %4, %0\n\t" \
+  "ds_read_b128 v[236:239], v224 offset:36864\n\t" \
+  "v_fmamk_f32 v206, v210, 0x3a84f106, v202\n\t" \
+  "v_fmamk_f32 v207, v211, 0x3a84f106, v202\n\t" \
+  "v_fmamk_f32 v214, v218, 0x3a84f106, v202\n\t" \
+  "v_fmamk_f32 v215, v219, 0x3a84f106, v202\n\t" \
+  "v_fmaak_f32 v210, v206, v210, 0xc0134593\n\t" \
+  "v_fmaak_f32 v211, v207, v211, 0xc0134593\n\t" \
+  "v_fmaak_f32 v218, v214, v218, 0xc0134593\n\t" \
+  "v_fmaak_f32 v219, v215, v219, 0xc0134593\n\t" \
+  "s_waitcnt lgkmcnt(6)\n\t" \
+  MN " %1, v[240:243], %4, %1\n\t" \
+  "ds_read_b128 v[240:243], v225 offset:32768\n\t" \
+  "v_mul_f32 v208, v208, v210\n\t" \
+  "v_mul_f32 v209, v209, v211\n\t" \
+  "v_mul_f32 v216, v216, v218\n\t" \
+  "v_mul_f32 v217, v217, v219\n\t" \
+  "v_exp_f32 v208, v208\n\t" \
+  "v_exp_f32 v209, v209\n\t" \
+  "v_exp_f32 v216, v216\n\t" \
+  "s_waitcnt lgkmcnt(6)\n\t" \
+  MN " %0, v[244:247], %5, %0\n\t" \
+  "ds_read_b128 v[244:247], v225 offset:36864\n\t" \
+  "v_exp_f32 v217, v217\n\t" \
+  "v_add_f32 v208, 1.0, v208\n\t" \
+  "v_add_f32 v209, 1.0, v209\n\t" \
+  "v_add_f32 v216, 1.0, v216\n\t" \
+  "v_add_f32 v217, 1.0, v217\n\t" \
+  "v_rcp_f32 v208, v208\n\t" \
+  "v_rcp_f32 v209, v209\n\t" \
+  "v_rcp_f32 v216, v216\n\t" \
+  "s_waitcnt lgkmcnt(6)\n\t" \
+  MN " %1, v[248:251], %5, %1\n\t" \
+  "ds_read_b128 v[248:251], v226 offset:32768\n\t" \
+  "v_rcp_f32 v217, v217\n\t" \
+  "v_accvgpr_read_b32 v206, a200\n\t" \
+  "v_accvgpr_read_b32 v207, a201\n\t" \
+  "v_accvgpr_read_b32 v214, a202\n\t" \
+  "v_accvgpr_read_b32 v215, a203\n\t" \
+  "v_fma_f32 v206, v220, v206, v176\n\t" \
+  "v_fma_f32 v207, v220, v207, v177\n\t" \
+  "v_fma_f32 v214, v220, v214, v178\n\t" \
+  "s_waitcnt lgkmcnt(6)\n\t" \
+  MN " %0, v[252:255], %6, %0\n\t" \
+  "ds_read_b128 v[252:255], v226 offset:36864\n\t" \
+  "v_fma_f32 v215, v220, v215, v179\n\t" \
+  "v_mul_f32 v204, v204, v208\n\t" \
+  "v_mul_f32 v205, v205, v209\n\t" \
+  "v_mul_f32 v212, v212, v216\n\t" \
+  "v_mul_f32 v213, v213, v217\n\t" \
+  "v_mul_f32 v206, v206, v204\n\t" \
+  "v_mul_f32 v207, v207, v205\n\t" \
+  "v_mul_f32 v214, v214, v212\n\t" \
+  "s_waitcnt lgkmcnt(6)\n\t" \
+  MN " %1, v[228:231], %6, %1\n\t" \
+  "ds_read_b128 v[228:231], v227 offset:32768\n\t" \
+  "v_mul_f32 v215, v215, v213\n\t" \
+  CVT " v156, v206, v207\n\t" \
+  CVT " v157, v214, v215\n\t" \
+  "v_accvgpr_read_b32 v204, a220\n\t" \
+  "v_accvgpr_read_b32 v205, a221\n\t" \
+  "v_accvgpr_read_b32 v212, a222\n\t" \
+  "v_accvgpr_read_b32 v213, a223\n\t" \
+  "s_waitcnt lgkmcnt(6)\n\t" \
+  MN " %0, v[232:235], %7, %0\n\t" \
+  "ds_read_b128 v[232:235], v227 offset:36864\n\t" \
+  "v_fma_f32 v204, v220, v204, v196\n\t" \
+  "v_fma_f32 v205, v220, v205, v197\n\t" \
+  "v_fma_f32 v212, v220, v212, v198\n\t" \
+  "v_fma_f32 v213, v220, v213, v199\n\t" \
+  "v_med3_f32 v208, v204, v201, v200\n\t" \
+  "v_med3_f32 v209, v205, v201, v200\n\t" \
+  "v_med3_f32 v216, v212, v201, v200\n\t" \
+  "v_med3_f32 v217, v213, v201, v200\n\t" \
+  "s_waitcnt lgkmcnt(6)\n\t" \
+  MN " %1, v[236:239], %7, %1\n\t" \
+  "v_mul_f32 v210, v208, v208\n\t" \
+  "v_mul_f32 v211, v209, v209\n\t" \
+  "v_mul_f32 v218, v216, v216\n\t" \
+  "v_mul_f32 v219, v217, v217\n\t" \
+  "v_fmamk_f32 v206, v210, 0x3a84f106, v202\n\t" \
+  "v_fmamk_f32 v207, v211, 0x3a84f106, v202\n\t" \
+  "v_fmamk_f32 v214, v218, 0x3a84f106, v202\n\t" \
+  "v_fmamk_f32 v215, v219, 0x3a84f106, v202\n\t" \
+  "s_waitcnt lgkmcnt(5)\n\t" \
+  MN " %0, v[240:243], %8, %0\n\t" \
+  "v_fmaak_f32 v210, v206, v210, 0xc0134593\n\t" \
+  "v_fmaak_f32 v211, v207, v211, 0xc0134593\n\t" \
+  "v_fmaak_f32 v218, v214, v218, 0xc0134593\n\t" \
+  "v_fmaak_f32 v219, v215, v219, 0xc0134593\n\t" \
+  "v_mul_f32 v208, v208, v210\n\t" \
+  "v_mul_f32 v209, v209, v211\n\t" \
+  "v_mul_f32 v216, v216, v218\n\t" \
+  "v_mul_f32 v217, v217, v219\n\t" \
+  "s_waitcnt lgkmcnt(4)\n\t" \
+  MN " %1, v[244:247], %8, %1\n\t" \
+  "v_exp_f32 v208, v208\n\t" \
+  "v_exp_f32 v209, v209\n\t" \
+  "v_exp_f32 v216, v216\n\t" \
+  "v_exp_f32 v217, v217\n\t" \
+  "v_add_f32 v208, 1.0, v208\n\t" \
+  "v_add_f32 v209, 1.0, v209\n\t" \
+  "v_add_f32 v216, 1.0, v216\n\t" \
+  "s_waitcnt lgkmcnt(3)\n\t" \
+  MN " %0, v[248:251], %9, %0\n\t" \
+  "v_add_f32 v217, 1.0, v217\n\t" \
+  "v_rcp_f32 v208, v208\n\t" \
+  "v_rcp_f32 v209, v209\n\t" \
+  "v_rcp_f32 v216, v216\n\t" \
+  "v_rcp_f32 v217, v217\n\t" \
+  "v_accvgpr_read_b32 v206, a204\n\t" \
+  "v_accvgpr_read_b32 v207, a205\n\t" \
+  "v_accvgpr_read_b32 v214, a206\n\t" \
+  "s_waitcnt lgkmcnt(2)\n\t" \
+  MN " %1, v[252:255], %9, %1\n\t" \
+  "v_accvgpr_read_b32 v215, a207\n\t" \
+  "v_fma_f32 v206, v220, v206, v180\n\t" \
+  "v_fma_f32 v207, v220, v207, v181\n\t" \
+  "v_fma_f32 v214, v220, v214, v182\n\t" \
+  "v_fma_f32 v215, v220, v215, v183\n\t" \
+  "v_mul_f32 v204, v204, v208\n\t" \
+  "v_mul_f32 v205, v205, v209\n\t" \
+  "v_mul_f32 v212, v212, v216\n\t" \
+  "s_waitcnt lgkmcnt(1)\n\t" \
+  MN " %0, v[228:231], %10, %0\n\t" \
+  "v_mul_f32 v213, v213, v217\n\t" \
+  "v_mul_f32 v206, v206, v204\n\t" \
+  "v_mul_f32 v207, v207, v205\n\t" \
+  "v_mul_f32 v214, v214, v212\n\t" \
+  "v_mul_f32 v215, v215, v213\n\t" \
+  CVT " v158, v206, v207\n\t" \
+  CVT " v159, v214, v215\n\t" \
+  "s_waitcnt lgkmcnt(0)\n\t" \
+  MN " %1, v[232:235], %10, %1\n\t" \
+  "s_nop 15\n\t"
+
+#define TC_ASM_FF2_E(MN, CVT) \
+  "v_add_u32 v224, %16, %17\n\t" \
+  "v_xor_b32 v225, 0x20, %17\n\t" \
+  "v_add_u32 v225, %16, v225\n\t" \
+  "v_xor_b32 v226, 0x40, %17\n\t" \
+  "v_add_u32 v226, %16, v226\n\t" \
+  "v_xor_b32 v227, 0x60, %17\n\t" \
+  "v_add_u32 v227, %16, v227\n\t" \
+  "v_mov_b32 v220, %27\n\t" \
+  "v_mov_b32 v200, 0x41000000\n\t" \
+  "v_mov_b32 v201, 0xc1000000\n\t" \
+  "v_mov_b32 v202, 0xbddaad3c\n\t" \
+  "s_waitcnt lgkmcnt(0)\n\t" \
+  "ds_read_b128 v[228:231], v224 offset:0\n\t" \
+  "ds_read_b128 v[232:235], v224 offset:4096\n\t" \
+  "ds_read_b128 v[236:239], v224 offset:8192\n\t" \
+  "ds_read_b128 v[240:243], v224 offset:12288\n\t" \
+  "ds_read_b128 v[244:247], v224 offset:16384\n\t" \
+  "ds_read_b128 v[248:251], v224 offset:20480\n\t" \
+  "ds_read_b128 v[252:255], v224 offset:24576\n\t" \
+  "s_waitcnt lgkmcnt(6)\n\t" \
+  MN " %0, v[228:231], %14, %0\n\t" \
+  "ds_read_b128 v[228:231], v224 offset:28672\n\t" \
+  "v_accvgpr_read_b32 v204, a240\n\t" \
+  "v_accvgpr_read_b32 v205, a241\n\t" \
+  "v_accvgpr_read_b32 v212, a242\n\t" \
+  "v_accvgpr_read_b32 v213, a243\n\t" \
+  "v_fma_f32 v204, v220, v204, v184\n\t" \
+  "v_fma_f32 v205, v220, v205, v185\n\t" \
+  "v_fma_f32 v212, v220, v212, v186\n\t" \
+  "v_fma_f32 v213, v220, v213, v187\n\t" \
+  "s_waitcnt lgkmcnt(6)\n\t" \
+  MN " %1, v[232:235], %14, %1\n\t" \
+  "ds_read_b128 v[232:235], v224 offset:32768\n\t" \
+  "v_med3_f32 v208, v204, v201, v200\n\t" \
+  "v_med3_f32 v209, v205, v201, v200\n\t" \
+  "v_med3_f32 v216, v212, v201, v200\n\t" \
+  "v_med3_f32 v217, v213, v201, v200\n\t" \
+  "v_mul_f32 v210, v208, v208\n\t" \
+  "v_mul_f32 v211, v209, v209\n\t" \
+  "v_mul_f32 v218, v216, v216\n\t" \
+  "v_mul_f32 v219, v217, v217\n\t" \
+  "s_waitcnt lgkmcnt(6)\n\t" \
+  MN " %2, v[236:239], %14, %2\n\t" \
+  "ds_read_b128 v[236:239], v224 offset:36864\n\t" \
+  "v_fmamk_f32 v206, v210, 0x3a84f106, v202\n\t" \
+  "v_fmamk_f32 v207, v211, 0x3a84f106, v202\n\t" \
+  "v_fmamk_f32 v214, v218, 0x3a84f106, v202\n\t" \
+  "v_fmamk_f32 v215, v219, 0x3a84f106, v202\n\t" \
+  "v_fmaak_f32 v210, v206, v210, 0xc0134593\n\t" \
+  "v_fmaak_f32 v211, v207, v211, 0xc0134593\n\t" \
+  "v_fmaak_f32 v218, v214, v218, 0xc0134593\n\t" \
+  "v_fmaak_f32 v219, v215, v219, 0xc0134593\n\t" \
+  "s_waitcnt lgkmcnt(6)\n\t" \
+  MN " %3, v[240:243], %14, %3\n\t" \
+  "ds_read_b128 v[240:243], v225 offset:0\n\t" \
+  "v_mul_f32 v208, v208, v210\n\t" \
+  "v_mul_f32 v209, v209, v211\n\t" \
+  "v_mul_f32 v216, v216, v218\n\t" \
+  "v_mul_f32 v217, v217, v219\n\t" \
+  "v_exp_f32 v208, v208\n\t" \
+  "v_exp_f32 v209, v209\n\t" \
+  "v_exp_f32 v216, v216\n\t" \
+  "v_exp_f32 v217, v217\n\t" \
+  "s_waitcnt lgkmcnt(6)\n\t" \
+  MN " %4, v[244:247], %14, %4\n\t" \
+  "ds_read_b128 v[244:247], v225 offset:4096\n\t" \
+  "v_add_f32 v208, 1.0, v208\n\t" \
+  "v_add_f32 v209, 1.0, v209\n\t" \
+  "v_add_f32 v216, 1.0, v216\n\t" \
+  "v_add_f32 v217, 1.0, v217\n\t" \
+  "v_rcp_f32 v208, v208\n\t" \
+  "v_rcp_f32 v209, v209\n\t" \
+  "v_rcp_f32 v216, v216\n\t" \
+  "v_rcp_f32 v217, v217\n\t" \
+  "s_waitcnt lgkmcnt(6)\n\t" \
+  MN " %5, v[248:251], %14, %5\n\t" \
+  "ds_read_b128 v[248:251], v225 offset:8192\n\t" \
+  "v_accvgpr_read_b32 v206, a224\n\t" \
+  "v_accvgpr_read_b32 v207, a225\n\t" \
+  "v_accvgpr_read_b32 v214, a226\n\t" \
+  "v_accvgpr_read_b32 v215, a227\n\t" \
+  "v_fma_f32 v206, v220, v206, v168\n\t" \
+  "v_fma_f32 v207, v220, v207, v169\n\t" \
+  "v_fma_f32 v214, v220, v214, v170\n\t" \
+  "v_fma_f32 v215, v220, v215, v171\n\t" \
+  "s_waitcnt lgkmcnt(6)\n\t" \
+  MN " %6, v[252:255], %14, %6\n\t" \
+  "ds_read_b128 v[252:255], v225 offset:12288\n\t" \
+  "v_mul_f32 v204, v204, v208\n\t" \
+  "v_mul_f32 v205, v205, v209\n\t" \
+  "v_mul_f32 v212, v212, v216\n\t" \
+  "v_mul_f32 v213, v213, v217\n\t" \
+  "v_mul_f32 v206, v206, v204\n\t" \
+  "v_mul_f32 v207, v207, v205\n\t" \
+  "v_mul_f32 v214, v214, v212\n\t" \
+  "v_mul_f32 v215, v215, v213\n\t" \
+  "s_waitcnt lgkmcnt(6)\n\t" \
+  MN " %7, v[228:231], %14, %7\n\t" \
+  "ds_read_b128 v[228:231], v225 offset:16384\n\t" \
+  CVT " v160, v206, v207\n\t" \
+  CVT " v161, v214, v215\n\t" \
+  "v_accvgpr_read_b32 v204, a244\n\t" \
+  "v_accvgpr_read_b32 v205, a245\n\t" \
+  "v_accvgpr_read_b32 v212, a246\n\t" \
+  "v_accvgpr_read_b32 v213, a247\n\t" \
+  "v_fma_f32 v204, v220, v204, v188\n\t" \
+  "v_fma_f32 v205, v220, v205, v189\n\t" \
+  "s_waitcnt lgkmcnt(6)\n\t" \
+  MN " %8, v[232:235], %14, %8\n\t" \
+  "ds_read_b128 v[232:235], v225 offset:20480\n\t" \
+  "v_fma_f32 v212, v220, v212, v190\n\t" \
+  "v_fma_f32 v213, v220, v213, v191\n\t" \
+  "v_med3_f32 v208, v204, v201, v200\n\t" \
+  "v_med3_f32 v209, v205, v201, v200\n\t" \
+  "v_med3_f32 v216, v212, v201, v200\n\t" \
+  "v_med3_f32 v217, v213, v201, v200\n\t" \
+  "v_mul_f32 v210, v208, v208\n\t" \
+  "v_mul_f32 v211, v209, v209\n\t" \
+  "s_waitcnt lgkmcnt(6)\n\t" \
+  MN " %9, v[236:239], %14, %9\n\t" \
+  "ds_read_b128 v[236:239], v225 offset:24576\n\t" \
+  "s_cmp_lg_u32 %20, 0\n\t" \
+  "s_cbranch_scc1 .Ltc%=_0\n\t" \
+  "s_mov_b32 m0, %13\n\t" \
+  "s_nop 0\n\t" \
+  "buffer_load_dwordx4 %18, %19, %12 offen offset:0 lds\n\t" \
+  "buffer_load_dwordx4 %18, %19, %12 offen offset:1024 lds\n\t" \
+  "buffer_load_dwordx4 %18, %19, %12 offen offset:2048 lds\n\t" \
+  "buffer_load_dwordx4 %18, %19, %12 offen offset:3072 lds\n\t" \
+  "s_add_u32 %12, %12, 0x1000\n\t" \
+  "s_add_u32 %13, %13, 0x1000\n\t" \
+  "s_mov_b32 m0, %13\n\t" \
+  "s_nop 0\n\t" \
+  "buffer_load_dwordx4 %18, %19, %12 offen offset:0 lds\n\t" \
+  "buffer_load_dwordx4 %18, %19, %12 offen offset:1024 lds\n\t" \
+  "buffer_load_dwordx4 %18, %19, %12 offen offset:2048 lds\n\t" \
+  "buffer_load_dwordx4 %18, %19, %12 offen offset:3072 lds\n\t" \
+  "s_add_u32 %12, %12, 0x1000\n\t" \
+  "s_add_u32 %13, %13, 0x1000\n\t" \
+  "s_mov_b32 m0, %13\n\t" \
+  "s_nop 0\n\t" \
+  "buffer_load_dwordx4 %18, %19, %12 offen offset:0 lds\n\t" \
+  "buffer_load_dwordx4 %18, %19, %12 offen offset:1024 lds\n\t" \
+  "buffer_load_dwordx4 %18, %19, %12 offen offset:2048 lds\n\t" \
+  ".Ltc%=_0:\n\t" \
+  "v_mul_f32 v218, v216, v216\n\t" \
+  "v_mul_f32 v219, v217, v217\n\t" \
+  "v_fmamk_f32 v206, v210, 0x3a84f106, v202\n\t" \
+  "v_fmamk_f32 v207, v211, 0x3a84f106, v202\n\t" \
+  "v_fmamk_f32 v214, v218, 0x3a84f106, v202\n\t" \
+  "v_fmamk_f32 v215, v219, 0x3a84f106, v202\n\t" \
+  "v_fmaak_f32 v210, v206, v210, 0xc0134593\n\t" \
+  "v_fmaak_f32 v211, v207, v211, 0xc0134593\n\t" \
+  "s_waitcnt lgkmcnt(6)\n\t" \
+  MN " %0, v[240:243], %15, %0\n\t" \
+  "ds_read_b128 v[240:243], v225 offset:28672\n\t" \
+  "v_fmaak_f32 v218, v214, v218, 0xc0134593\n\t" \
+  "v_fmaak_f32 v219, v215, v219, 0xc0134593\n\t" \
+  "v_mul_f32 v208, v208, v210\n\t" \
+  "v_mul_f32 v209, v209, v211\n\t" \
+  "v_mul_f32 v216, v216, v218\n\t" \
+  "v_mul_f32 v217, v217, v219\n\t" \
+  "v_exp_f32 v208, v208\n\t" \
+  "v_exp_f32 v209, v209\n\t" \
+  "s_waitcnt lgkmcnt(6)\n\t" \
+  MN " %1, v[244:247], %15, %1\n\t" \
+  "ds_read_b128 v[244:247], v225 offset:32768\n\t" \
+  "v_exp_f32 v216, v216\n\t" \
+  "v_exp_f32 v217, v217\n\t" \
+  "v_add_f32 v208, 1.0, v208\n\t" \
+  "v_add_f32 v209, 1.0, v209\n\t" \
+  "v_add_f32 v216, 1.0, v216\n\t" \
+  "v_add_f32 v217, 1.0, v217\n\t" \
+  "v_rcp_f32 v208, v208\n\t" \
+  "v_rcp_f32 v209, v209\n\t" \
+  "s_waitcnt lgkmcnt(6)\n\t" \
+  MN " %2, v[248:251], %15, %2\n\t" \
+  "ds_read_b128 v[248:251], v225 offset:36864\n\t" \
+  "v_rcp_f32 v216, v216\n\t" \
+  "v_rcp_f32 v217, v217\n\t" \
+  "v_accvgpr_read_b32 v206, a228\n\t" \
+  "v_accvgpr_read_b32 v207, a229\n\t" \
+  "v_accvgpr_read_b32 v214, a230\n\t" \
+  "v_accvgpr_read_b32 v215, a231\n\t" \
+  "v_fma_f32 v206, v220, v206, v172\n\t" \
+  "v_fma_f32 v207, v220, v207, v173\n\t" \
+  "s_waitcnt lgkmcnt(6)\n\t" \
+  MN " %3, v[252:255], %15, %3\n\t" \
+  "ds_read_b128 v[252:255], v226 offset:0\n\t" \
+  "v_fma_f32 v214, v220, v214, v174\n\t" \
+  "v_fma_f32 v215, v220, v215, v175\n\t" \
+  "v_mul_f32 v204, v204, v208\n\t" \
+  "v_mul_f32 v205, v205, v209\n\t" \
+  "v_mul_f32 v212, v212, v216\n\t" \
+  "v_mul_f32 v213, v213, v217\n\t" \
+  "v_mul_f32 v206, v206, v204\n\t" \
+  "v_mul_f32 v207, v207, v205\n\t" \
+  "s_waitcnt lgkmcnt(6)\n\t" \
+  MN " %4, v[228:231], %15, %4\n\t" \
+  "ds_read_b128 v[228:231], v226 offset:4096\n\t" \
+  "v_mul_f32 v214, v214, v212\n\t" \
+  "v_mul_f32 v215, v215, v213\n\t" \
+  CVT " v162, v206, v207\n\t" \
+  CVT " v163, v214, v215\n\t" \
+  "v_accvgpr_read_b32 v204, a248\n\t" \
+  "v_accvgpr_read_b32 v205, a249\n\t" \
+  "v_accvgpr_read_b32 v212, a250\n\t" \
+  "v_accvgpr_read_b32 v213, a251\n\t" \
+  "s_waitcnt lgkmcnt(6)\n\t" \
+  MN " %5, v[232:235], %15, %5\n\t" \
+  "ds_read_b128 v[232:235], v226 offset:8192\n\t" \
+  "v_fma_f32 v204, v220, v204, v192\n\t" \
+  "v_fma_f32 v205, v220, v205, v193\n\t" \
+  "v_fma_f32 v212, v220, v212, v194\n\t" \
+  "v_fma_f32 v213, v220, v213, v195\n\t" \
+  "v_med3_f32 v208, v204, v201, v200\n\t" \
+  "v_med3_f32 v209, v205, v201, v200\n\t" \
+  "v_med3_f32 v216, v212, v201, v200\n\t" \
+  "v_med3_f32 v217, v213, v201, v200\n\t" \
+  "s_waitcnt lgkmcnt(6)\n\t" \
+  MN " %6, v[236:239], %15, %6\n\t" \
+  "ds_read_b128 v[236:239], v226 offset:12288\n\t" \
+  "v_mul_f32 v210, v208, v208\n\t" \
+  "v_mul_f32 v211, v209, v209\n\t" \
+  "v_mul_f32 v218, v216, v216\n\t" \
+  "v_mul_f32 v219, v217, v217\n\t" \
+  "v_fmamk_f32 v206, v210, 0x3a84f106, v202\n\t" \
+  "v_fmamk_f32 v207, v211, 0x3a84f106, v202\n\t" \
+  "v_fmamk_f32 v214, v218, 0x3a84f106, v202\n\t" \
+  "v_fmamk_f32 v215, v219, 0x3a84f106, v202\n\t" \
+  "s_waitcnt lgkmcnt(6)\n\t" \
+  MN " %7, v[240:243], %15, %7\n\t" \
+  "ds_read_b128 v[240:243], v226 offset:16384\n\t" \
+  "v_fmaak_f32 v210, v206, v210, 0xc0134593\n\t" \
+  "v_fmaak_f32 v211, v207, v211, 0xc0134593\n\t" \
+  "v_fmaak_f32 v218, v214, v218, 0xc0134593\n\t" \
+  "v_fmaak_f32 v219, v215, v219, 0xc0134593\n\t" \
+  "v_mul_f32 v208, v208, v210\n\t" \
+  "v_mul_f32 v209, v209, v211\n\t" \
+  "v_mul_f32 v216, v216, v218\n\t" \
+  "v_mul_f32 v217, v217, v219\n\t" \
+  "s_waitcnt lgkmcnt(6)\n\t" \
+  MN " %8, v[244:247], %15, %8\n\t" \
+  "ds_read_b128 v[244:247], v226 offset:20480\n\t" \
+  "v_exp_f32 v208, v208\n\t" \
+  "v_exp_f32 v209, v209\n\t" \
+  "v_exp_f32 v216, v216\n\t" \
+  "v_exp_f32 v217, v217\n\t" \
+  "v_add_f32 v208, 1.0, v208\n\t" \
+  "v_add_f32 v209, 1.0, v209\n\t" \
+  "v_add_f32 v216, 1.0, v216\n\t" \
+  "v_add_f32 v217, 1.0, v217\n\t" \
+  "s_waitcnt lgkmcnt(6)\n\t" \
+  MN " %9, v[248:251], %15, %9\n\t" \
+  "ds_read_b128 v[248:251], v226 offset:24576\n\t" \
+  "s_cmp_lg_u32 %20, 1\n\t" \
+  "s_cbranch_scc1 .Ltc%=_1\n\t" \
+  "s_mov_b32 m0, %13\n\t" \
+  "s_nop 0\n\t" \
+  "buffer_load_dwordx4 %18, %19, %12 offen offset:0 lds\n\t" \
+  "buffer_load_dwordx4 %18, %19, %12 offen offset:1024 lds\n\t" \
+  "buffer_load_dwordx4 %18, %19, %12 offen offset:2048 lds\n\t" \
+  "buffer_load_dwordx4 %18, %19, %12 offen offset:3072 lds\n\t" \
+  "s_add_u32 %12, %12, 0x1000\n\t" \
+  "s_add_u32 %13, %13, 0x1000\n\t" \
+  "s_mov_b32 m0, %13\n\t" \
+  "s_nop 0\n\t" \
+  "buffer_load_dwordx4 %18, %19, %12 offen offset:0 lds\n\t" \
+  "buffer_load_dwordx4 %18, %19, %12 offen offset:1024 lds\n\t" \
+  "buffer_load_dwordx4 %18, %19, %12 offen offset:2048 lds\n\t" \
+  "buffer_load_dwordx4 %18, %19, %12 offen offset:3072 lds\n\t" \
+  "s_add_u32 %12, %12, 0x1000\n\t" \
+  "s_add_u32 %13, %13, 0x1000\n\t" \
+  "s_mov_b32 m0, %13\n\t" \
+  "s_nop 0\n\t" \
+  "buffer_load_dwordx4 %18, %19, %12 offen offset:0 lds\n\t" \
+  "buffer_load_dwordx4 %18, %19, %12 offen offset:1024 lds\n\t" \
+  "buffer_load_dwordx4 %18, %19, %12 offen offset:2048 lds\n\t" \
+  ".Ltc%=_1:\n\t" \
+  "v_rcp_f32 v208, v208\n\t" \
+  "v_rcp_f32 v209, v209\n\t" \
+  "v_rcp_f32 v216, v216\n\t" \
+  "v_rcp_f32 v217, v217\n\t" \
+  "v_accvgpr_read_b32 v206, a232\n\t" \
+  "v_accvgpr_read_b32 v207, a233\n\t" \
+  "v_accvgpr_read_b32 v214, a234\n\t" \
+  "v_accvgpr_read_b32 v215, a235\n\t" \
+  "s_waitcnt lgkmcnt(6)\n\t" \
+  "s_nop 1\n\t" \
+  MN " %0, v[252:255], %10, %0\n\t" \
+  "ds_read_b128 v[252:255], v226 offset:28672\n\t" \
+  "v_fma_f32 v206, v220, v206, v176\n\t" \
+  "v_fma_f32 v207, v220, v207, v177\n\t" \
+  "v_fma_f32 v214, v220, v214, v178\n\t" \
+  "v_fma_f32 v215, v220, v215, v179\n\t" \
+  "v_mul_f32 v204, v204, v208\n\t" \
+  "v_mul_f32 v205, v205, v209\n\t" \
+  "v_mul_f32 v212, v212, v216\n\t" \
+  "v_mul_f32 v213, v213, v217\n\t" \
+  "s_waitcnt lgkmcnt(6)\n\t" \
+  MN " %1, v[228:231], %10, %1\n\t" \
+  "ds_read_b128 v[228:231], v226 offset:32768\n\t" \
+  "v_mul_f32 v206, v206, v204\n\t" \
+  "v_mul_f32 v207, v207, v205\n\t" \
+  "v_mul_f32 v214, v214, v212\n\t" \
+  "v_mul_f32 v215, v215, v213\n\t" \
+  CVT " v164, v206, v207\n\t" \
+  CVT " v165, v214, v215\n\t" \
+  "v_accvgpr_read_b32 v204, a252\n\t" \
+  "v_accvgpr_read_b32 v205, a253\n\t" \
+  "s_waitcnt lgkmcnt(6)\n\t" \
+  MN " %2, v[232:235], %10, %2\n\t" \
+  "ds_read_b128 v[232:235], v226 offset:36864\n\t" \
+  "v_accvgpr_read_b32 v212, a254\n\t" \
+  "v_accvgpr_read_b32 v213, a255\n\t" \
+  "v_fma_f32 v204, v220, v204, v196\n\t" \
+  "v_fma_f32 v205, v220, v205, v197\n\t" \
+  "v_fma_f32 v212, v220, v212, v198\n\t" \
+  "v_fma_f32 v213, v220, v213, v199\n\t" \
+  "v_med3_f32 v208, v204, v201, v200\n\t" \
+  "v_med3_f32 v209, v205, v201, v200\n\t" \
+  "s_waitcnt lgkmcnt(6)\n\t" \
+  MN " %3, v[236:239], %10, %3\n\t" \
+  "ds_read_b128 v[236:239], v227 offset:0\n\t" \
+  "v_med3_f32 v216, v212, v201, v200\n\t" \
+  "v_med3_f32 v217, v213, v201, v200\n\t" \
+  "v_mul_f32 v210, v208, v208\n\t" \
+  "v_mul_f32 v211, v209, v209\n\t" \
+  "v_mul_f32 v218, v216, v216\n\t" \
+  "v_mul_f32 v219, v217, v217\n\t" \
+  "v_fmamk_f32 v206, v210, 0x3a84f106, v202\n\t" \
+  "v_fmamk_f32 v207, v211, 0x3a84f106, v202\n\t" \
+  "s_waitcnt lgkmcnt(6)\n\t" \
+  MN " %4, v[240:243], %10, %4\n\t" \
+  "ds_read_b128 v[240:243], v227 offset:4096\n\t" \
+  "v_fmamk_f32 v214, v218, 0x3a84f106, v202\n\t" \
+  "v_fmamk_f32 v215, v219, 0x3a84f106, v202\n\t" \
+  "v_fmaak_f32 v210, v206, v210, 0xc0134593\n\t" \
+  "v_fmaak_f32 v211, v207, v211, 0xc0134593\n\t" \
+  "v_fmaak_f32 v218, v214, v218, 0xc0134593\n\t" \
+  "v_fmaak_f32 v219, v215, v219, 0xc0134593\n\t" \
+  "v_mul_f32 v208, v208, v210\n\t" \
+  "v_mul_f32 v209, v209, v211\n\t" \
+  "s_waitcnt lgkmcnt(6)\n\t" \
+  MN " %5, v[244:247], %10, %5\n\t" \
+  "ds_read_b128 v[244:247], v227 offset:8192\n\t" \
+  "v_mul_f32 v216, v216, v218\n\t" \
+  "v_mul_f32 v217, v217, v219\n\t" \
+  "v_exp_f32 v208, v208\n\t" \
+  "v_exp_f32 v209, v209\n\t" \
+  "v_exp_f32 v216, v216\n\t" \
+  "v_exp_f32 v217, v217\n\t" \
+  "v_add_f32 v208, 1.0, v208\n\t" \
+  "v_add_f32 v209, 1.0, v209\n\t" \
+  "s_waitcnt lgkmcnt(6)\n\t" \
+  MN " %6, v[248:251], %10, %6\n\t" \
+  "ds_read_b128 v[248:251], v227 offset:12288\n\t" \
+  "v_add_f32 v216, 1.0, v216\n\t" \
+  "v_add_f32 v217, 1.0, v217\n\t" \
+  "v_rcp_f32 v208, v208\n\t" \
+  "v_rcp_f32 v209, v209\n\t" \
+  "v_rcp_f32 v216, v216\n\t" \
+  "v_rcp_f32 v217, v217\n\t" \
+  "v_accvgpr_read_b32 v206, a236\n\t" \
+  "v_accvgpr_read_b32 v207, a237\n\t" \
+  "s_waitcnt lgkmcnt(6)\n\t" \
+  MN " %7, v[252:255], %10, %7\n\t" \
+  "ds_read_b128 v[252:255], v227 offset:16384\n\t" \
+  "v_accvgpr_read_b32 v214, a238\n\t" \
+  "v_accvgpr_read_b32 v215, a239\n\t" \
+  "v_fma_f32 v206, v220, v206, v180\n\t" \
+  "v_fma_f32 v207, v220, v207, v181\n\t" \
+  "v_fma_f32 v214, v220, v214, v182\n\t" \
+  "v_fma_f32 v215, v220, v215, v183\n\t" \
+  "v_mul_f32 v204, v204, v208\n\t" \
+  "v_mul_f32 v205, v205, v209\n\t" \
+  "s_waitcnt lgkmcnt(6)\n\t" \
+  MN " %8, v[228:231], %10, %8\n\t" \
+  "ds_read_b128 v[228:231], v227 offset:20480\n\t" \
+  "v_mul_f32 v212, v212, v216\n\t" \
+  "v_mul_f32 v213, v213, v217\n\t" \
+  "v_mul_f32 v206, v206, v204\n\t" \
+  "v_mul_f32 v207, v207, v205\n\t" \
+  "v_mul_f32 v214, v214, v212\n\t" \
+  "v_mul_f32 v215, v215, v213\n\t" \
+  CVT " v166, v206, v207\n\t" \
+  CVT " v167, v214, v215\n\t" \
+  "s_waitcnt lgkmcnt(6)\n\t" \
+  MN " %9, v[232:235], %10, %9\n\t" \
+  "ds_read_b128 v[232:235], v227 offset:24576\n\t" \
+  "s_cmp_lg_u32 %20, 2\n\t" \
+  "s_cbranch_scc1 .Ltc%=_2\n\t" \
+  "s_mov_b32 m0, %13\n\t" \
+  "s_nop 0\n\t" \
+  "buffer_load_dwordx4 %18, %19, %12 offen offset:0 lds\n\t" \
+  "buffer_load_dwordx4 %18, %19, %12 offen offset:1024 lds\n\t" \
+  "buffer_load_dwordx4 %18, %19, %12 offen offset:2048 lds\n\t" \
+  "buffer_load_dwordx4 %18, %19, %12 offen offset:3072 lds\n\t" \
+  "s_add_u32 %12, %12, 0x1000\n\t" \
+  "s_add_u32 %13, %13, 0x1000\n\t" \
+  "s_mov_b32 m0, %13\n\t" \
+  "s_nop 0\n\t" \
+  "buffer_load_dwordx4 %18, %19, %12 offen offset:0 lds\n\t" \
+  "buffer_load_dwordx4 %18, %19, %12 offen offset:1024 lds\n\t" \
+  "buffer_load_dwordx4 %18, %19, %12 offen offset:2048 lds\n\t" \
+  "buffer_load_dwordx4 %18, %19, %12 offen offset:3072 lds\n\t" \
+  "s_add_u32 %12, %12, 0x1000\n\t" \
+  "s_add_u32 %13, %13, 0x1000\n\t" \
+  "s_mov_b32 m0, %13\n\t" \
+  "s_nop 0\n\t" \
+  "buffer_load_dwordx4 %18, %19, %12 offen offset:0 lds\n\t" \
+  "buffer_load_dwordx4 %18, %19, %12 offen offset:1024 lds\n\t" \
+  "buffer_load_dwordx4 %18, %19, %12 offen offset:2048 lds\n\t" \
+  ".Ltc%=_2:\n\t" \
+  "s_waitcnt lgkmcnt(6)\n\t" \
+  "s_nop 1\n\t" \
+  MN " %0, v[236:239], %11, %0\n\t" \
+  "ds_read_b128 v[236:239], v227 offset:28672\n\t" \
+  "s_waitcnt lgkmcnt(6)\n\t" \
+  MN " %1, v[240:243], %11, %1\n\t" \
+  "ds_read_b128 v[240:243], v227 offset:32768\n\t" \
+  "s_waitcnt lgkmcnt(6)\n\t" \
+  MN " %2, v[244:247], %11, %2\n\t" \
+  "ds_read_b128 v[244:247], v227 offset:36864\n\t" \
+  "s_waitcnt lgkmcnt(6)\n\t" \
+  MN " %3, v[248:251], %11, %3\n\t" \
+  "s_waitcnt lgkmcnt(5)\n\t" \
+  MN " %4, v[252:255], %11, %4\n\t" \
+  "s_waitcnt lgkmcnt(4)\n\t" \
+  MN " %5, v[228:231], %11, %5\n\t" \
+  "s_waitcnt lgkmcnt(3)\n\t" \
+  MN " %6, v[232:235], %11, %6\n\t" \
+  "s_waitcnt lgkmcnt(2)\n\t" \
+  MN " %7, v[236:239], %11, %7\n\t" \
+  "s_waitcnt lgkmcnt(1)\n\t" \
+  MN " %8, v[240:243], %11, %8\n\t" \
+  "s_waitcnt lgkmcnt(0)\n\t" \
+  MN " %9, v[244:247], %11, %9\n\t" \
+  "s_cmp_lg_u32 %20, 3\n\t" \
+  "s_cbranch_scc1 .Ltc%=_3\n\t" \
+  "s_mov_b32 m0, %13\n\t" \
+  "s_nop 0\n\t" \
+  "buffer_load_dwordx4 %18, %19, %12 offen offset:0 lds\n\t" \
+  "buffer_load_dwordx4 %18, %19, %12 offen offset:1024 lds\n\t" \
+  "buffer_load_dwordx4 %18, %19, %12 offen offset:2048 lds\n\t" \
+  "buffer_load_dwordx4 %18, %19, %12 offen offset:3072 lds\n\t" \
+  "s_add_u32 %12, %12, 0x1000\n\t" \
+  "s_add_u32 %13, %13, 0x1000\n\t" \
+  "s_mov_b32 m0, %13\n\t" \
+  "s_nop 0\n\t" \
+  "buffer_load_dwordx4 %18, %19, %12 offen offset:0 lds\n\t" \
+  "buffer_load_dwordx4 %18, %19, %12 offen offset:1024 lds\n\t" \
+  "buffer_load_dwordx4 %18, %19, %12 offen offset:2048 lds\n\t" \
+  "buffer_load_dwordx4 %18, %19, %12 offen offset:3072 lds\n\t" \
+  "s_add_u32 %12, %12, 0x1000\n\t" \
+  "s_add_u32 %13, %13, 0x1000\n\t" \
+  "s_mov_b32 m0, %13\n\t" \
+  "s_nop 0\n\t" \
+  "buffer_load_dwordx4 %18, %19, %12 offen offset:0 lds\n\t" \
+  "buffer_load_dwordx4 %18, %19, %12 offen offset:1024 lds\n\t" \
+  "buffer_load_dwordx4 %18, %19, %12 offen offset:2048 lds\n\t" \
+  ".Ltc%=_3:\n\t" \
+  "s_nop 15\n\t"
+
+#define TC_FF_HID0 "{v[152:155]}"
+#define TC_FF_HID1 "{v[156:159]}"
+#define TC_FF_HID2 "{v[160:163]}"
+#define TC_FF_HID3 "{v[164:167]}"
+#define TC_FF_TA0 "{v[168:175]}"
+#define TC_FF_TG0 "{v[184:191]}"
+#define TC_FF_TA1 "{v[176:183]}"
+#define TC_FF_TG1 "{v[192:199]}"
+#define TC_FF_AG0A "{a[192:207]}"
+#define TC_FF_AG0G "{a[208:223]}"
+#define TC_FF_AG1A "{a[224:239]}"
+#define TC_FF_AG1G "{a[240:255]}"
+#define TC_FF_CLOBBERS "v200", "v201", "v202", "v203", "v204", "v205", "v206", "v207", "v208", "v209", "v210", "v211", "v212", "v213", "v214", "v215", "v216", "v217", "v218", "v219", "v220", "v221", "v222", "v223", "v224", "v225", "v226", "v227", "v228", "v229", "v230", "v231", "v232", "v233", "v234", "v235", "v236", "v237", "v238", "v239", "v240", "v241", "v242", "v243", "v244", "v245", "v246", "v247", "v248", "v249", "v250", "v251", "v252", "v253", "v254", "v255"
```

Result: no change. 29.37 images/s (-0.0%).
